# tulip-control/polytope

Measured on AMD Instinct MI355X. Metric: LP solves/sec (batched Chebyshev + redundancy), higher is better.
Workload: dtype f64

## Files before the change

### polytope_amd/csrc/plp_bbox_lane.hip

```cpp
#include "plp_reduce_lane.hpp"

namespace plp {

template <int D>
static int launch_bbox_lane_d(long long B, int m_max, const double* A, const double* b, const int* mrows, double* lb, double* ub,
                              int* status, hipStream_t st, double* xfin) {
    if (B > 2147483647ll) return 1;
    const int force = 0;
    const bool wide = m_max > LN_ROWS;
    int gs = wide ? (B <= PLP_REDUCE_LANE32_GS16_MAXB ? 16 : 8) : (B <= PLP_REDUCE_LANE_GS16_MAXB ? 16 : (B <= PLP_REDUCE_LANE_GS8_MAXB ? 8 : 4));
    const long long ng = 64 / gs;
    long long blocks = (B + ng - 1) / ng;
    if (blocks < 1) blocks = 1;
#define PLP_BBL(GSV, RV)                                                                                                     \
    hipLaunchKernelGGL((bbox_lane_kernel<D, GSV, RV>), dim3((unsigned)blocks), dim3(RBLOCK), reduce_lane_smem_bytes(D, GSV, RV), st, B, \
                       m_max, A, b, mrows, force, lb, ub, status, xfin)
    if (wide) { if (gs == 16) PLP_BBL(16, 32); else PLP_BBL(8, 32); }
    else if (gs == 16) PLP_BBL(16, 16);
    else if (gs == 8) PLP_BBL(8, 16);
    else PLP_BBL(4, 16);
#undef PLP_BBL
    return 0;
}

int launch_bbox_lane(long long B, int m_max, int d, const double* A, const double* b, const int* mrows, double* lb, double* ub,
                     int* status, hipStream_t st, double* xfin) {
    if (m_max < 1 || m_max > 2 * LN_ROWS) return 1;
    switch (d) {
        case 1: return launch_bbox_lane_d<1>(B, m_max, A, b, mrows, lb, ub, status, st, xfin);
        case 2: return launch_bbox_lane_d<2>(B, m_max, A, b, mrows, lb, ub, status, st, xfin);
        case 3: return launch_bbox_lane_d<3>(B, m_max, A, b, mrows, lb, ub, status, st, xfin);
        default: return 1;
    }
}

}
```

### polytope_amd/csrc/plp_kernels.hpp

```cpp
#pragma once
#include "plp_common.hpp"

namespace plp {

static inline int group_size_for(int m_max) {
    if (m_max < 0 || m_max > MAX_M) return -1;
    if (m_max <= 8) return 8;
    if (m_max <= 16) return 16;
    if (m_max <= 32) return 32;
    return 64;
}

int launch_lp(long long B, int m_max, int n, const double* c, const double* G, const double* h, const int* mrows,
              double* x, double* fun, int* status, int* iters, hipStream_t st);
int launch_lp_phase(long long B, int m_max, int n, const double* c, const double* G, const double* h, const int* mrows,
                    double* x, double* fun, int* status, int* iters, hipStream_t st, int phase, int* more);

int launch_cheby(long long B, int m_max, int d, const double* A, const double* b, const int* mrows, double* r,
                 double* xc, int* status, hipStream_t st);

int launch_lp_lds(long long B, int m_max, int n, const double* c, const double* G, const double* h, const int* mrows,
                  double* x, double* fun, int* status, int* iters, hipStream_t st);
int launch_cheby_lds(long long B, int m_max, int d, const double* A, const double* b, const int* mrows, double* r,
                     double* xc, int* status, hipStream_t st);
size_t lds_lp_bytes(int m_max, int nc);

int launch_cheby_gather_r(int d, long long n0, long long n1, long long n2, const int* off, const int* rows, const int* sel,
                          const double* A, const double* b, double* out, hipStream_t st);
int launch_rdiff_server(int d, int nwg, const unsigned long long* mail, const int* rec, void* out, unsigned long long* alive,
                        unsigned long long* dstate, const double* A, const double* b, unsigned long long last_word,
                        unsigned idle_polls, hipStream_t st);
void launch_rdiff_publish(long long n, const double* src, double* host_out, unsigned long long* host_flag,
                          unsigned long long seq, hipStream_t st);
int launch_cheby_gather_w(int d, long long nlp, const int* off, const int* rows, const int* sel, const double* A,
                          const double* b, double* out, hipStream_t st);
int launch_cheby_gather_lds(int d, int m_cap, long long nlp, const int* off, const int* rows, const int* sel,
                            const double* A, const double* b, double* out, hipStream_t st);

int launch_fm(int emit, long long B, int m_max, int d, const double* A, const double* b, const int* mrows,
              const unsigned long long* keep, int kw, const int* flags, int col, int first, double abs_tol, int* count,
              int mo_max, double* Aout, double* bout, int* mout, hipStream_t st);
size_t fm_lds_bytes(int m_max, int d);
int launch_volume_hits(long long B, int m_max, int d, const double* A, const double* b, const int* mrows, const double* lb,
                       const double* ub, const unsigned long long* state, const unsigned long long* inc, long long N,
                       unsigned* hits, int* flags, hipStream_t st);
int launch_support(long long B, int m_max, int d, const double* A, const double* b, const int* mrows, int K, const double* C,
                   int c_shared, const double* xc, double* val, double* x, int* status, hipStream_t st);
int launch_reduce_lds(long long B, int m_max, int d, const double* A, const double* b, const int* mrows, double abs_tol,
                      unsigned long long* keep, int* flags, double* r, double* xc, int* nlp, hipStream_t st);

int launch_cheby_w(long long B, int m_max, int d, const double* A, const double* b, const int* mrows, double* r,
                   double* xc, int* status, hipStream_t st);

int launch_lp_w(long long B, int m_max, int n, const double* c, const double* G, const double* h, const int* mrows,
                double* x, double* fun, int* status, int* iters, hipStream_t st);

int launch_lp_r(long long B, int m_max, int n, const double* c, const double* G, const double* h, const int* mrows,
                double* x, double* fun, int* status, int* iters, hipStream_t st);

int launch_cheby_r(long long B, int m_max, int d, const double* A, const double* b, const int* mrows, double* r,
                   double* xc, int* status, hipStream_t st);

struct BoxHandover {
    signed char* basis8;
    double* centre;
    double* xfin;
    int mode;
};
int launch_bbox(long long B, int m_max, int d, const double* A, const double* b, const int* mrows, double* lb,
                double* ub, int* status, hipStream_t st, BoxHandover* ho = nullptr);
int launch_bbox_lazy(long long B, int m_max, int d, const double* A, const double* b, const int* mrows, double* lb,
                     double* ub, int* status, hipStream_t st, BoxHandover* ho = nullptr);

int launch_adjacent(int n, int m_max, int d, const double* A, const double* b, const int* mrows, double inflate,
                    double thresh, unsigned char* adj, long long p_lo, long long p_hi, unsigned char* compact,
                    hipStream_t st, int cross_n1 = 0);

int launch_adjacent_w(int n, int m_max, int d, const double* A, const double* b, const int* mrows, double inflate,
                      double thresh, unsigned char* adj, long long p_lo, long long p_hi, unsigned char* compact,
                      hipStream_t st, int cross_n1 = 0);

struct ReduceArgs {
    long long B;
    int m_max;
    const double* A;
    const double* b;
    const int* mrows;
    double abs_tol;
    unsigned long long* keep;
    int* flags;
    double* r;
    double* xc;
    int* nlp;
    unsigned long long* ctr;
    unsigned long long* retry_word;
    unsigned long long epoch;
};
int launch_reduce(int d, const ReduceArgs& a, int phase, hipStream_t st);

int launch_contains(int P, int m_max, int d, const double* A, const double* b, const int* mrows, long long N,
                    const double* X, double abs_tol, int mode, unsigned char* out, void* scratch, hipStream_t st);
size_t contains_scratch_bytes(int P, int m_max);

int launch_assign(long long N, int d, const double* X, int F, const double* normals, const double* offsets,
                  double abs_tol, int* facet_of_point, double* dist, long long* argmax, double* maxd,
                  void* scratch, size_t scratch_bytes, hipStream_t st);
size_t assign_scratch_bytes(long long N, int F);

int launch_hull_reassign(long long N, int d, const double* X, int* owner, double* dist, const unsigned char* dead,
                         int new_id0, int n_new, const double* normals, const double* offsets, double abs_tol,
                         long long* argmax, double* maxd, long long* count, hipStream_t st);
void launch_hull_mark(int n, const int* ids, unsigned char* dead, hipStream_t st);
void launch_hull_drop(long long n, const long long* idx, int* owner, hipStream_t st);

int launch_selftest(int gs, double* out_d, unsigned* out_u, hipStream_t st);

size_t verify_scratch_bytes(long long nlp, int m_max);
bool verify_enabled();
int launch_verify_lp(long long B, int m_max, int n, const double* c, const double* G, const double* h, const int* mrows,
                     double* x, double* fun, int* status, void* scratch, int parity, hipStream_t st);
int launch_verify_cheby(long long B, int m_max, int d, const double* A, const double* b, const int* mrows, double* r,
                        double* xc, int* status, void* scratch, int parity, hipStream_t st);
int launch_verify_box(long long B, int m_max, int d, const double* A, const double* b, const int* mrows, double* lb, double* ub,
                      int* status, const signed char* basis8, const double* centre, const double* xfin, void* scratch,
                      int parity, hipStream_t st);

}
```

### polytope_amd/csrc/plp_lane_lp.hpp

```cpp
#pragma once
#include <math.h>

#if defined(__HIPCC__)
#include "plp_common.hpp"
#define PLP_LANE_FN __device__ __forceinline__
#else
#define PLP_LANE_FN static inline
namespace plp {
enum : int { ST_OPT = 0, ST_ITER = 1, ST_INFEAS = 2, ST_UNBND = 3, ST_NUM = 4 };
constexpr int ST_RETRY = 5;
constexpr double TOL_D = 1e-9, TOL_PIV = 1e-7, DEGEN_EPS = 1e-12;
constexpr int BLAND_AFTER = 6;
}
#endif

namespace plp {
namespace lane {

constexpr int LANE_MAX_ITERS = 48;
constexpr double LANE_TOL_D = 1e-11, LANE_TOL_PIV = 1e-11;
constexpr double LANE_M_NOISE = 64 * 2.220446049250313e-16;

struct Lp3 {
    double x0, x1, x2;
    int w0, w1, w2;
    int nact;
    int status;
    int iters;
    int ndeg;
};

PLP_LANE_FN void cross3(double a0, double a1, double a2, double b0, double b1, double b2, double& e0, double& e1,
                        double& e2) {
    e0 = fma(a1, b2, -(a2 * b1));
    e1 = fma(a2, b0, -(a0 * b2));
    e2 = fma(a0, b1, -(a1 * b0));
}

PLP_LANE_FN double dot3(double a0, double a1, double a2, double b0, double b1, double b2) {
    return fma(a2, b2, fma(a1, b1, a0 * b0));
}

template <class AnyF>
PLP_LANE_FN void proj1(const double c0, const double c1, const double c2, const double cn1, const double n0, const double n1,
                       const double n2, const double nn, double& d0, double& d1, double& d2, double& scale, AnyF ANY) {
    const double cn = dot3(c0, c1, c2, n0, n1, n2);
    d0 = fma(cn, n0, -(nn * c0));
    d1 = fma(cn, n1, -(nn * c1));
    d2 = fma(cn, n2, -(nn * c2));
    scale = nn;
    const double pn1 = fabs(d0) + fabs(d1) + fabs(d2);
    const bool small = (pn1 > 0.0) & (pn1 < 1e-4 * (nn * cn1));
    if (ANY(small)) {
        const double np_ = dot3(n0, n1, n2, d0, d1, d2);
        const double q0 = fma(nn, d0, -(np_ * n0)), q1 = fma(nn, d1, -(np_ * n1)), q2 = fma(nn, d2, -(np_ * n2));
        d0 = small ? q0 : d0;
        d1 = small ? q1 : d1;
        d2 = small ? q2 : d2;
        scale = small ? nn * nn : nn;
    }
}

constexpr double LANE_PAIR_SIN2 = 1e-10;

template <class RowF, class RatioF, class Ratio0F, class AnyF>
PLP_LANE_FN void walk3(Lp3& S, const double c0, const double c1, const double c2, const bool go, RowF ROWS, RatioF RATIO,
                       Ratio0F RATIO0, AnyF ANY, const bool warm = false) {
    if (!warm) {
        S.x0 = S.x1 = S.x2 = 0.0;
        S.w0 = S.w1 = S.w2 = -1;
        S.nact = 0;
        S.iters = 0;
        S.ndeg = 0;
    }
    S.status = go ? -1 : ST_OPT;
    const double cn1 = fabs(c0) + fabs(c1) + fabs(c2);
    if (go && !(cn1 > 0.0)) S.status = ST_OPT;
    if (!warm && ANY(S.status < 0)) {
        const bool step = S.status < 0;
        const double d0 = -c0, d1 = -c1, d2 = -c2;
        const double tolp = LANE_TOL_PIV * cn1;
        double bs = 1.0, bd = 0.0;
        int bi = -1;
        RATIO0(d0, d1, d2, tolp, bs, bd, bi);
        if (step) {
            S.iters = 1;
            if (bi < 0) {
                S.status = ST_UNBND;
            } else {
                const double t = bs / bd;
                S.x0 = fma(t, d0, 0.0);
                S.x1 = fma(t, d1, 0.0);
                S.x2 = fma(t, d2, 0.0);
                S.w0 = bi;
                S.nact = 1;
                S.ndeg = (t * cn1 <= DEGEN_EPS) ? 1 : 0;
            }
        }
    }
    while (ANY(S.status < 0)) {
        const bool run = S.status < 0;
        double d0 = -c0, d1 = -c1, d2 = -c2;
        double n00 = 0, n01 = 0, n02 = 0, n10 = 0, n11 = 0, n12 = 0, n20 = 0, n21 = 0, n22 = 0;
        if (ANY(run && S.nact >= 1)) {
            if (S.nact >= 1) ROWS(S.w0, n00, n01, n02);
            if (S.nact >= 2) ROWS(S.w1, n10, n11, n12);
            if (S.nact >= 3) ROWS(S.w2, n20, n21, n22);
        }
        bool stalled = false;
        double dscale = cn1;
        if (S.nact == 1) {
            const double nn = dot3(n00, n01, n02, n00, n01, n02);
            double sc;
            proj1(c0, c1, c2, cn1, n00, n01, n02, nn, d0, d1, d2, sc, ANY);
            dscale = sc * cn1;
        } else if (S.nact == 2) {
            double e0, e1, e2;
            cross3(n00, n01, n02, n10, n11, n12, e0, e1, e2);
            const double ce = dot3(c0, c1, c2, e0, e1, e2);
            d0 = -(ce * e0);
            d1 = -(ce * e1);
            d2 = -(ce * e2);
            dscale = dot3(e0, e1, e2, e0, e1, e2) * cn1;
            const double nn0 = dot3(n00, n01, n02, n00, n01, n02), nn1 = dot3(n10, n11, n12, n10, n11, n12);
            if (run && !(dot3(e0, e1, e2, e0, e1, e2) > LANE_PAIR_SIN2 * nn0 * nn1)) S.status = ST_RETRY;
        } else if (S.nact == 3) {
            d0 = d1 = d2 = 0.0;
        }
        {
            const double dn1 = fabs(d0) + fabs(d1) + fabs(d2);
            stalled = !(dn1 > LANE_TOL_D * dscale);
        }
        if (ANY(S.status < 0 && stalled)) {
            if (S.status < 0 && stalled) {
                if (S.nact == 0) {
                    S.status = ST_OPT;
                } else if (S.nact == 1) {
                    const double cn = dot3(c0, c1, c2, n00, n01, n02);
                    if (cn <= 0.0) S.status = ST_OPT;
                    else { S.nact = 0; d0 = -c0; d1 = -c1; d2 = -c2; }
                } else if (S.nact == 2) {
                    const double g00 = dot3(n00, n01, n02, n00, n01, n02), g11 = dot3(n10, n11, n12, n10, n11, n12);
                    const double g01 = dot3(n00, n01, n02, n10, n11, n12);
                    const double r0 = -dot3(c0, c1, c2, n00, n01, n02), r1 = -dot3(c0, c1, c2, n10, n11, n12);
                    const double l0 = fma(r0, g11, -(r1 * g01)), l1 = fma(r1, g00, -(r0 * g01));
                    const double w0 = 0.5 * (1.0 + g00), w1 = 0.5 * (1.0 + g11);
                    const double tol0 = LANE_TOL_D * g11 * w0 * cn1, tol1 = LANE_TOL_D * g00 * w1 * cn1;
                    if (l0 >= -tol0 && l1 >= -tol1) S.status = ST_OPT;
                    else {
                        const bool drop0 = l0 * w0 < l1 * w1;
                        if (drop0) { S.w0 = S.w1; n00 = n10; n01 = n11; n02 = n12; }
                        S.nact = 1;
                        double sc;
                        proj1(c0, c1, c2, cn1, n00, n01, n02, dot3(n00, n01, n02, n00, n01, n02), d0, d1, d2, sc, [](bool q) { return q; });
                    }
                } else {
                    double u00, u01, u02, u10, u11, u12, u20, u21, u22;
                    cross3(n10, n11, n12, n20, n21, n22, u00, u01, u02);
                    cross3(n20, n21, n22, n00, n01, n02, u10, u11, u12);
                    cross3(n00, n01, n02, n10, n11, n12, u20, u21, u22);
                    const double det = dot3(n00, n01, n02, u00, u01, u02);
                    const double g00 = dot3(n00, n01, n02, n00, n01, n02), g11 = dot3(n10, n11, n12, n10, n11, n12);
                    const double g22 = dot3(n20, n21, n22, n20, n21, n22);
                    if (!(det * det > 1e-18 * (g00 * g11 * g22))) {
                        S.status = ST_RETRY;
                    } else {
                        const double sg = det > 0.0 ? 1.0 : -1.0;
                        const double l0 = -sg * dot3(c0, c1, c2, u00, u01, u02);
                        const double l1 = -sg * dot3(c0, c1, c2, u10, u11, u12);
                        const double l2 = -sg * dot3(c0, c1, c2, u20, u21, u22);
                        const double a0 = l0 * (0.5 * (1.0 + g00)), a1 = l1 * (0.5 * (1.0 + g11)), a2 = l2 * (0.5 * (1.0 + g22));
                        const double tol = LANE_TOL_D * fabs(det) * cn1;
                        if (a0 >= -tol && a1 >= -tol && a2 >= -tol) S.status = ST_OPT;
                        else {
                            int j = 0;
                            double am = a0;
                            if (a1 < am) { am = a1; j = 1; }
                            if (a2 < am) { am = a2; j = 2; }
                            double gg;
                            if (j == 0) { d0 = -sg * u00; d1 = -sg * u01; d2 = -sg * u02; S.w0 = S.w1; S.w1 = S.w2; gg = g11 * g22; }
                            else if (j == 1) { d0 = -sg * u10; d1 = -sg * u11; d2 = -sg * u12; S.w1 = S.w2; gg = g22 * g00; }
                            else { d0 = -sg * u20; d1 = -sg * u21; d2 = -sg * u22; gg = g00 * g11; }
                            S.nact = 2;
                            if (!(dot3(d0, d1, d2, d0, d1, d2) > LANE_PAIR_SIN2 * gg)) S.status = ST_RETRY;
                        }
                    }
                }
            }
        }
        const bool step = S.status < 0;
        const double dn1 = fabs(d0) + fabs(d1) + fabs(d2);
        const double tolp = LANE_TOL_PIV * dn1;
        double bs = 1.0, bd = 0.0;
        int bi = -1;
        if (ANY(step)) RATIO(d0, d1, d2, S.x0, S.x1, S.x2, tolp, bs, bd, bi);
        if (step) {
            ++S.iters;
            if (bi < 0) {
                S.status = ST_UNBND;
            } else {
                const double t = bs / bd;
                S.x0 = fma(t, d0, S.x0);
                S.x1 = fma(t, d1, S.x1);
                S.x2 = fma(t, d2, S.x2);
                if (S.nact == 0) S.w0 = bi;
                else if (S.nact == 1) S.w1 = bi;
                else S.w2 = bi;
                S.nact += 1;
                S.ndeg = (t * dn1 <= DEGEN_EPS) ? S.ndeg + 1 : 0;
                if (S.ndeg >= BLAND_AFTER || S.iters >= LANE_MAX_ITERS) S.status = ST_RETRY;
            }
        }
    }
}

template <class RowF, class RatioF, class AnyF>
PLP_LANE_FN void walk3(Lp3& S, const double c0, const double c1, const double c2, const bool go, RowF ROWS, RatioF RATIO,
                       AnyF ANY, const bool warm = false) {
    walk3(S, c0, c1, c2, go, ROWS, RATIO,
          [&](double d0, double d1, double d2, double tolp, double& bs, double& bd, int& bi) {
              RATIO(d0, d1, d2, 0.0, 0.0, 0.0, tolp, bs, bd, bi);
          },
          ANY, warm);
}

struct Lp4 {
    double x0, x1, x2, x3;
    int w0, w1, w2, w3;
    int nact, status, iters, ndeg;
};

PLP_LANE_FN double dot4(double a0, double a1, double a2, double a3, double b0, double b1, double b2, double b3) {
    return fma(a3, b3, fma(a2, b2, fma(a1, b1, a0 * b0)));
}

PLP_LANE_FN void gcross4(double p0, double p1, double p2, double p3, double q0, double q1, double q2, double q3, double r0,
                         double r1, double r2, double r3, double& e0, double& e1, double& e2, double& e3) {
    const double m01 = fma(q0, r1, -(q1 * r0)), m02 = fma(q0, r2, -(q2 * r0)), m03 = fma(q0, r3, -(q3 * r0));
    const double m12 = fma(q1, r2, -(q2 * r1)), m13 = fma(q1, r3, -(q3 * r1)), m23 = fma(q2, r3, -(q3 * r2));
    e0 = fma(p1, m23, fma(-p2, m13, p3 * m12));
    e1 = -fma(p0, m23, fma(-p2, m03, p3 * m02));
    e2 = fma(p0, m13, fma(-p1, m03, p3 * m01));
    e3 = -fma(p0, m12, fma(-p1, m02, p2 * m01));
}

template <class RowF, class RatioF, class AnyF>
PLP_LANE_FN void walk4(Lp4& S, const double c0, const double c1, const double c2, const double c3, const bool go, RowF ROWS,
                       RatioF RATIO, AnyF ANY) {
    S.x0 = S.x1 = S.x2 = S.x3 = 0.0;
    S.w0 = S.w1 = S.w2 = S.w3 = -1;
    S.nact = 0;
    S.iters = 0;
    S.ndeg = 0;
    S.status = go ? -1 : ST_OPT;
    const double cn1 = fabs(c0) + fabs(c1) + fabs(c2) + fabs(c3);
    if (go && !(cn1 > 0.0)) S.status = ST_OPT;
    while (ANY(S.status < 0)) {
        const bool run = S.status < 0;
        bool dropped = false;
        double d0 = -c0, d1 = -c1, d2 = -c2, d3 = -c3;
        double n00 = 0, n01 = 0, n02 = 0, n03 = 0, n10 = 0, n11 = 0, n12 = 0, n13 = 0;
        double n20 = 0, n21 = 0, n22 = 0, n23 = 0, n30 = 0, n31 = 0, n32 = 0, n33 = 0;
        if (ANY(run && S.nact >= 1)) {
            if (S.nact >= 1) ROWS(S.w0, n00, n01, n02, n03);
            if (S.nact >= 2) ROWS(S.w1, n10, n11, n12, n13);
            if (S.nact >= 3) ROWS(S.w2, n20, n21, n22, n23);
            if (S.nact >= 4) ROWS(S.w3, n30, n31, n32, n33);
        }
        const double g00 = dot4(n00, n01, n02, n03, n00, n01, n02, n03), g11 = dot4(n10, n11, n12, n13, n10, n11, n12, n13);
        const double g22 = dot4(n20, n21, n22, n23, n20, n21, n22, n23);
        const double g01 = dot4(n00, n01, n02, n03, n10, n11, n12, n13), g02 = dot4(n00, n01, n02, n03, n20, n21, n22, n23);
        const double g12 = dot4(n10, n11, n12, n13, n20, n21, n22, n23);
        const double r0 = dot4(c0, c1, c2, c3, n00, n01, n02, n03), r1 = dot4(c0, c1, c2, c3, n10, n11, n12, n13);
        const double r2 = dot4(c0, c1, c2, c3, n20, n21, n22, n23);
        double det = 1.0, m0 = 0.0, m1 = 0.0, m2 = 0.0;
        if (S.nact == 1) {
            det = g00;
            m0 = r0;
        } else if (S.nact == 2) {
            det = fma(g00, g11, -(g01 * g01));
            m0 = fma(r0, g11, -(r1 * g01));
            m1 = fma(r1, g00, -(r0 * g01));
            if (run && !(det > LANE_PAIR_SIN2 * g00 * g11)) S.status = ST_RETRY;
        } else if (S.nact == 3) {
            const double A00 = fma(g11, g22, -(g12 * g12)), A01 = fma(g02, g12, -(g01 * g22)), A02 = fma(g01, g12, -(g02 * g11));
            const double A11 = fma(g00, g22, -(g02 * g02)), A12 = fma(g01, g02, -(g00 * g12)), A22 = fma(g00, g11, -(g01 * g01));
            det = fma(g00, A00, fma(g01, A01, g02 * A02));
            m0 = fma(A00, r0, fma(A01, r1, A02 * r2));
            m1 = fma(A01, r0, fma(A11, r1, A12 * r2));
            m2 = fma(A02, r0, fma(A12, r1, A22 * r2));
            if (run && !(det > 1e-16 * g00 * g11 * g22)) S.status = ST_RETRY;
        }
        bool twice = false;
        if (S.nact == 3) {
            double e0, e1, e2, e3;
            gcross4(n00, n01, n02, n03, n10, n11, n12, n13, n20, n21, n22, n23, e0, e1, e2, e3);
            const double ce = dot4(c0, c1, c2, c3, e0, e1, e2, e3);
            d0 = -(ce * e0);
            d1 = -(ce * e1);
            d2 = -(ce * e2);
            d3 = -(ce * e3);
        } else if (S.nact >= 1 && S.nact <= 2) {
            d0 = fma(m1, n10, fma(m0, n00, -(det * c0)));
            d1 = fma(m1, n11, fma(m0, n01, -(det * c1)));
            d2 = fma(m1, n12, fma(m0, n02, -(det * c2)));
            d3 = fma(m1, n13, fma(m0, n03, -(det * c3)));
            if (S.nact == 1) {
                const double nd = dot4(n00, n01, n02, n03, d0, d1, d2, d3);
                d0 = fma(g00, d0, -(nd * n00));
                d1 = fma(g00, d1, -(nd * n01));
                d2 = fma(g00, d2, -(nd * n02));
                d3 = fma(g00, d3, -(nd * n03));
            } else {
                const double dn = fabs(d0) + fabs(d1) + fabs(d2) + fabs(d3);
                twice = (dn > 0.0) & (dn < 1e-4 * (det * cn1));
                if (ANY(run && twice)) {
                    const double s0 = dot4(d0, d1, d2, d3, n00, n01, n02, n03), s1 = dot4(d0, d1, d2, d3, n10, n11, n12, n13);
                    const double k0 = fma(s0, g11, -(s1 * g01)), k1 = fma(s1, g00, -(s0 * g01));
                    const double q0 = fma(det, d0, -fma(k1, n10, k0 * n00)), q1 = fma(det, d1, -fma(k1, n11, k0 * n01));
                    const double q2 = fma(det, d2, -fma(k1, n12, k0 * n02)), q3 = fma(det, d3, -fma(k1, n13, k0 * n03));
                    d0 = twice ? q0 : d0;
                    d1 = twice ? q1 : d1;
                    d2 = twice ? q2 : d2;
                    d3 = twice ? q3 : d3;
                }
            }
        } else if (S.nact == 4) {
            d0 = d1 = d2 = d3 = 0.0;
        }
        const double dscale = (S.nact >= 1 && S.nact <= 3) ? ((S.nact == 1 || twice) ? det * det : det) * cn1 : cn1;
        const bool stalled = !(fabs(d0) + fabs(d1) + fabs(d2) + fabs(d3) > LANE_TOL_D * dscale);
        if (ANY(S.status < 0 && stalled)) {
            if (S.status < 0 && stalled) {
                const double w0 = 0.5 * (1.0 + g00), w1 = 0.5 * (1.0 + g11), w2 = 0.5 * (1.0 + g22);
                if (S.nact == 0) {
                    S.status = ST_OPT;
                } else if (S.nact <= 3) {
                    const double tol = LANE_TOL_D * det * cn1;
                    double f0 = 0.0, f1 = 0.0, f2 = 0.0;
                    if (S.nact == 2) {
                        f0 = fabs(r0 * g11) + fabs(r1 * g01);
                        f1 = fabs(r1 * g00) + fabs(r0 * g01);
                    } else if (S.nact == 3) {
                        const double B00 = fabs(g11 * g22) + g12 * g12, B01 = fabs(g02 * g12) + fabs(g01 * g22), B02 = fabs(g01 * g12) + fabs(g02 * g11);
                        const double B11 = fabs(g00 * g22) + g02 * g02, B12 = fabs(g01 * g02) + fabs(g00 * g12), B22 = fabs(g00 * g11) + g01 * g01;
                        f0 = B00 * fabs(r0) + B01 * fabs(r1) + B02 * fabs(r2);
                        f1 = B01 * fabs(r0) + B11 * fabs(r1) + B12 * fabs(r2);
                        f2 = B02 * fabs(r0) + B12 * fabs(r1) + B22 * fabs(r2);
                    }
                    const double a0 = -m0 * w0, a1 = S.nact >= 2 ? -m1 * w1 : 0.0, a2 = S.nact >= 3 ? -m2 * w2 : 0.0;
                    const double t0 = fmax(tol, LANE_M_NOISE * f0 * w0), t1 = fmax(tol, LANE_M_NOISE * f1 * w1), t2 = fmax(tol, LANE_M_NOISE * f2 * w2);
                    if (a0 >= -t0 && a1 >= -t1 && a2 >= -t2) {
                        S.status = ST_OPT;
                    } else {
                        int j = 0;
                        double am = a0 + t0;
                        if (a1 + t1 < am) { am = a1 + t1; j = 1; }
                        if (a2 + t2 < am) { am = a2 + t2; j = 2; }
                        if (j == 0) S.w0 = S.w1;
                        if (j <= 1) S.w1 = S.w2;
                        S.nact -= 1;
                        dropped = true;
                    }
                } else {
                    const double g33 = dot4(n30, n31, n32, n33, n30, n31, n32, n33);
                    const double w3 = 0.5 * (1.0 + g33);
                    double am = 0.0, bd0 = 0.0, bd1 = 0.0, bd2 = 0.0, bd3 = 0.0, dj_abs = 0.0;
                    int jbest = -1;
                    bool all_ok = true, singular = false;
#define PLP_W4_VERTEX(J, P, Q, R, NJ0, NJ1, NJ2, NJ3, WJ)                                                          \
                    {                                                                                                   \
                        double u0, u1, u2, u3;                                                                          \
                        gcross4(P##0, P##1, P##2, P##3, Q##0, Q##1, Q##2, Q##3, R##0, R##1, R##2, R##3, u0, u1, u2, u3); \
                        const double dj = dot4(NJ0, NJ1, NJ2, NJ3, u0, u1, u2, u3);                                     \
                        const double sg = dj > 0.0 ? 1.0 : -1.0;                                                        \
                        const double lj = -sg * dot4(c0, c1, c2, c3, u0, u1, u2, u3);                                   \
                        const double aj = lj * (WJ);                                                                    \
                        dj_abs = fabs(dj);                                                                              \
                        singular = singular | !(dj * dj > 1e-18 * (g00 * g11 * g22 * g33));                            \
                        all_ok = all_ok & (aj >= -(LANE_TOL_D * dj_abs * cn1));                                              \
                        const bool better = (jbest < 0) | (aj < am);                                                    \
                        am = better ? aj : am;                                                                          \
                        jbest = better ? (J) : jbest;                                                                   \
                        bd0 = better ? -sg * u0 : bd0;                                                                  \
                        bd1 = better ? -sg * u1 : bd1;                                                                  \
                        bd2 = better ? -sg * u2 : bd2;                                                                  \
                        bd3 = better ? -sg * u3 : bd3;                                                                  \
                    }
                    PLP_W4_VERTEX(0, n1, n2, n3, n00, n01, n02, n03, w0)
                    PLP_W4_VERTEX(1, n0, n2, n3, n10, n11, n12, n13, w1)
                    PLP_W4_VERTEX(2, n0, n1, n3, n20, n21, n22, n23, w2)
                    PLP_W4_VERTEX(3, n0, n1, n2, n30, n31, n32, n33, w3)
#undef PLP_W4_VERTEX
                    if (singular) S.status = ST_RETRY;
                    else if (all_ok) S.status = ST_OPT;
                    else {
                        d0 = bd0; d1 = bd1; d2 = bd2; d3 = bd3;
                        if (jbest == 0) S.w0 = S.w1;
                        if (jbest <= 1) S.w1 = S.w2;
                        if (jbest <= 2) S.w2 = S.w3;
                        S.nact = 3;
                    }
                }
            }
        }
        if (dropped) {
            ++S.iters;
            if (S.iters >= LANE_MAX_ITERS) S.status = ST_RETRY;
        }
        const bool step = (S.status < 0) & !dropped;
        const double dn1 = fabs(d0) + fabs(d1) + fabs(d2) + fabs(d3);
        const double tolp = LANE_TOL_PIV * dn1;
        double bs = 1.0, bd = 0.0;
        int bi = -1;
        if (ANY(step)) RATIO(d0, d1, d2, d3, S.x0, S.x1, S.x2, S.x3, tolp, bs, bd, bi);
        if (step) {
            ++S.iters;
            if (bi < 0) {
                S.status = ST_UNBND;
            } else {
                const double t = bs / bd;
                S.x0 = fma(t, d0, S.x0);
                S.x1 = fma(t, d1, S.x1);
                S.x2 = fma(t, d2, S.x2);
                S.x3 = fma(t, d3, S.x3);
                if (S.nact == 0) S.w0 = bi;
                else if (S.nact == 1) S.w1 = bi;
                else if (S.nact == 2) S.w2 = bi;
                else S.w3 = bi;
                S.nact += 1;
                S.ndeg = (t * dn1 <= DEGEN_EPS) ? S.ndeg + 1 : 0;
                if (S.ndeg >= BLAND_AFTER || S.iters >= LANE_MAX_ITERS) S.status = ST_RETRY;
            }
        }
    }
}

PLP_LANE_FN void ratio_row4(const double a0, const double a1, const double a2, const double a3, const double beta, const int i,
                            const double d0, const double d1, const double d2, const double d3, const double x0,
                            const double x1, const double x2, const double x3, const double tolp, double& bs, double& bd,
                            int& bi) {
    const double ad = dot4(a0, a1, a2, a3, d0, d1, d2, d3);
    const double ax = dot4(a0, a1, a2, a3, x0, x1, x2, x3);
    const double sl = fmax(beta - ax, 0.0);
    const bool better = (ad > tolp) & (sl * bd < bs * ad);
    bs = better ? sl : bs;
    bd = better ? ad : bd;
    bi = better ? i : bi;
}

PLP_LANE_FN void ratio_row(const double a0, const double a1, const double a2, const double beta, const int i, const double d0,
                           const double d1, const double d2, const double x0, const double x1, const double x2,
                           const double tolp, double& bs, double& bd, int& bi) {
    const double ad = dot3(a0, a1, a2, d0, d1, d2);
    const double ax = dot3(a0, a1, a2, x0, x1, x2);
    const double sl = fmax(beta - ax, 0.0);
    const bool better = (ad > tolp) & (sl * bd < bs * ad);
    bs = better ? sl : bs;
    bd = better ? ad : bd;
    bi = better ? i : bi;
}

PLP_LANE_FN void ratio_row0(const double a0, const double a1, const double a2, const double beta, const int i, const double d0,
                            const double d1, const double d2, const double tolp, double& bs, double& bd, int& bi) {
    const double ad = dot3(a0, a1, a2, d0, d1, d2);
    const double sl = fmax(beta, 0.0);
    const bool better = (ad > tolp) & (sl * bd < bs * ad);
    bs = better ? sl : bs;
    bd = better ? ad : bd;
    bi = better ? i : bi;
}

template <int M, class RowF, class BetaF, class AnyF, class PassF>
PLP_LANE_FN void solve3(Lp3& S, const double c0, const double c1, const double c2, const bool go, RowF ROWS, BetaF BETA,
                        AnyF ANY, PassF PASS, const bool warm = false) {
    walk3(S, c0, c1, c2, go, ROWS,
          [&](double d0, double d1, double d2, double x0, double x1, double x2, double tolp, double& bs, double& bd, int& bi) {
              PASS();
#pragma unroll
              for (int i = 0; i < M; ++i) {
                  double a0, a1, a2;
                  ROWS(i, a0, a1, a2);
                  ratio_row(a0, a1, a2, BETA(i), i, d0, d1, d2, x0, x1, x2, tolp, bs, bd, bi);
              }
          },
          ANY, warm);
}

template <int M, class RowF, class BetaF, class AnyF>
PLP_LANE_FN void solve3(Lp3& S, const double c0, const double c1, const double c2, const bool go, RowF ROWS, BetaF BETA,
                        AnyF ANY, const bool warm = false) {
    solve3<M>(S, c0, c1, c2, go, ROWS, BETA, ANY, [] {}, warm);
}

}
}
```

### polytope_amd/csrc/plp_reduce.hip

```cpp
#include "plp_kernels.hpp"
#include "plp_reduce_plan.hpp"

namespace plp {

template <int D>
int launch_reduce_d(const ReduceLaunch& L, const ReduceArgs& a, int force, int retry_only, hipStream_t st);

static int launch_plan(int d, const ReduceLaunch& L, const ReduceArgs& a, int force, int retry_only, hipStream_t st) {
    switch (d) {
#define PLP_CASE_D(K) \
    case K: return launch_reduce_d<K>(L, a, force, retry_only, st);
        PLP_CASE_D(1) PLP_CASE_D(2) PLP_CASE_D(3) PLP_CASE_D(4) PLP_CASE_D(5) PLP_CASE_D(6) PLP_CASE_D(7) PLP_CASE_D(8)
        PLP_CASE_D(9) PLP_CASE_D(10) PLP_CASE_D(11) PLP_CASE_D(12) PLP_CASE_D(13) PLP_CASE_D(14) PLP_CASE_D(15) PLP_CASE_D(16)
#undef PLP_CASE_D
        default: return 2;
    }
}

int launch_reduce(int d, const ReduceArgs& a, int phase, hipStream_t st) {
    const ReducePlan p = plan_reduce(a.B, a.m_max, d, reduce_env());
    if (p.first.engine == RE_NONE) return 2;
    if (phase != 2) {
        const int rc = launch_plan(d, p.first, a, p.force_retry, 0, st);
        if (rc || !p.second || phase == 1) return rc;
    }
    return launch_plan(d, p.retry, a, p.force_retry, 1, st);
}

}
```

### polytope_amd/csrc/plp_reduce_d1_4.hip

```cpp
#include "plp_reduce_launch.hpp"

namespace plp {

PLP_REDUCE_INSTANTIATE(1)
PLP_REDUCE_INSTANTIATE(2)
PLP_REDUCE_INSTANTIATE(3)
PLP_REDUCE_INSTANTIATE(4)

}

#ifdef PLP_STAGE_STATS
extern "C" __attribute__((visibility("default"))) int plp_debug_stage_stats(unsigned long long* out16, int reset) {
    (void)hipDeviceSynchronize();
    if (out16 && hipMemcpyFromSymbol(out16, HIP_SYMBOL(plp::plp_stage_stats), 128) != hipSuccess) return 1;
    if (reset) {
        unsigned long long z[16] = {0};
        if (hipMemcpyToSymbol(HIP_SYMBOL(plp::plp_stage_stats), z, 128) != hipSuccess) return 1;
    }
    return 0;
}
#endif
```

### polytope_amd/csrc/plp_reduce_lane.hpp

```cpp
#pragma once
#include <type_traits>

#include "plp_lane_lp.hpp"
#include "plp_reduce_general.hpp"
#include "plp_reduce_r_impl.hpp"

namespace plp {

#ifndef PLP_LANE_CH
#define PLP_LANE_CH 4
#endif

constexpr int LN_ROWS = 16;

template <int D, int GS, int ROWS>
__device__ __noinline__ void reduce_lane_redo(unsigned char* smem_raw, const long long tile, const int ntile, const uint64_t rb64,
                                              int m_max, const double* __restrict__ Ag, const double* __restrict__ bg,
                                              const int* __restrict__ mrows, double abs_tol,
                                              unsigned long long* __restrict__ keep_out, int* __restrict__ flags_out,
                                              double* __restrict__ r_out, double* __restrict__ xc_out,
                                              int* __restrict__ nlp_out) {
    constexpr int PER = 64 / ROWS;
    for (int sub = 0; sub < (64 / GS) / PER; ++sub) {
        unsigned some = 0u;
#pragma unroll
        for (int q = 0; q < PER; ++q) some |= (unsigned)((rb64 >> (GS * (PER * sub + q))) & 1ull) << q;
        if (some == 0u) continue;
        const int q = (threadIdx.x & 63) / ROWS;
        const bool mine = ((some >> q) & 1u) != 0u;
        const int left = ntile - PER * sub;
        reduce_general_tile<D, RBLOCK>(smem_raw, tile + PER * sub, left < PER ? left : PER, mine, m_max, ROWS, Ag, bg, mrows, abs_tol,
                                       keep_out, flags_out, r_out, xc_out, nlp_out);
    }
}

template <int D, int GS, int ROWS = LN_ROWS, bool BBOX = false>
__device__ __forceinline__ void reduce_lane_tile(
    const long long tile, long long B, int m_max, const double* __restrict__ Ag, const double* __restrict__ bg,
    const int* __restrict__ mrows, double abs_tol, int force_retry, unsigned long long* __restrict__ keep_out,
    int* __restrict__ flags_out, double* __restrict__ r_out, double* __restrict__ xc_out, int* __restrict__ nlp_out,
    unsigned long long* __restrict__ ctr) {
    static_assert(D >= 1 && D <= 4, "the lane engine walks in R^3 (lower dimensions are embedded) or R^4");
    static_assert(RBLOCK == 64, "one wavefront per workgroup");
    static_assert(GS == 4 || GS == 8 || GS == 16, "lanes per polytope");
    static_assert((ROWS == 16 || ROWS == 32) && ROWS / GS >= 1 && ROWS / GS <= 4, "row slots per polytope, at most four per lane");
    constexpr int rows = ROWS, R = rows / GS, NG = 64 / GS;
    constexpr unsigned RMASK = (1u << R) - 1u;
    constexpr int LS = NG;
    extern __shared__ __attribute__((aligned(16))) unsigned char smem_raw[];
    const Grp g(GS);
    const int lane = g.lane;
    const int gib = lane / GS;
    const int row0 = g.gl * R;
    double* sA = reinterpret_cast<double*>(smem_raw);
    double* sb = sA + (size_t)rows * D * NG;
    double* san = sb + (size_t)rows * NG;
    double* myA = sA + gib;
    constexpr int OFF_B = rows * D * NG, OFF_N = OFF_B + rows * NG;
    double* const myb = myA + OFF_B;
    double* const myan = myA + OFF_N;
#define LA(i, kk) myA[((i) * D + (kk)) * LS]
#define LB(i) myA[OFF_B + (i) * LS]
#define LN(i) myA[OFF_N + (i) * LS]
    double* const rA = myA + row0 * D * LS;
    double* const rS = myA + row0 * LS;
#define OA(k, kk) rA[((k) * D + (kk)) * LS]
#define OB(k) rS[OFF_B + (k) * LS]
#define ON(k) rS[OFF_N + (k) * LS]
    const double qnan = __longlong_as_double(0x7ff8000000000000ll);
    const double pinf = __longlong_as_double(0x7ff0000000000000ll);
    const int ntile = (B - tile) < NG ? (int)(B - tile) : NG;
    __syncthreads();
    {
        const int p = lane % NG, q = lane / NG;
        const int rowsz = m_max * D;
        const bool pv = p < ntile;
        const double* src = Ag + (tile + (pv ? p : 0)) * rowsz;
        double va[rows * D / GS], vb[rows / GS];
        const double* srcb = bg + (tile + (pv ? p : 0)) * m_max;
        if (m_max == rows) {
#pragma unroll
            for (int it = 0; it < rows * D / GS; ++it) va[it] = src[q + GS * it];
#pragma unroll
            for (int it = 0; it < rows / GS; ++it) vb[it] = srcb[q + GS * it];
        } else {
#pragma unroll
            for (int it = 0; it < rows * D / GS; ++it) {
                const int rem = q + GS * it;
                va[it] = src[rem < rowsz ? rem : 0];
            }
#pragma unroll
            for (int it = 0; it < rows / GS; ++it) {
                const int row = q + GS * it;
                vb[it] = srcb[row < m_max ? row : 0];
            }
        }
#pragma unroll
        for (int it = 0; it < rows * D / GS; ++it) {
            const int rem = q + GS * it;
            sA[rem * NG + p] = (pv & (rem < rowsz)) ? va[it] : 0.0;
        }
#pragma unroll
        for (int it = 0; it < rows / GS; ++it) {
            const int row = q + GS * it;
            sb[row * NG + p] = (pv & (row < m_max)) ? vb[it] : 0.0;
        }
    }
    __syncthreads();
    const bool valid = gib < ntile;
    const int m = valid ? (mrows ? (mrows + tile)[gib] : m_max) : 0;
    double xc[D];
    double rr = 0.0;
    bool ball, fulldim, f1open = false;
    uint64_t live = 0ull;
    unsigned has = 0u;
    bool retry = force_retry != 0;
    {
        SimplexR<D + 1, R, false, true> S;
        double qi[R];
        S.reset(D + 1, m, row0);
        unsigned actb = 0u;
        bool inf0 = false, finite = true;
#pragma unroll
        for (int k = 0; k < R; ++k) {
            const bool h = valid & (row0 + k < m) & (m <= rows);
            has |= h ? (1u << k) : 0u;
            double nrm2 = 0.0;
#pragma unroll
            for (int kk = 0; kk < D; ++kk) {
                const double v = h ? OA(k, kk) : 0.0;
                S.T[k][kk] = v;
                nrm2 = nrm2 + v * v;
                finite = finite & isfinite(v);
            }
            const double bk = h ? OB(k) : 0.0;
            finite = finite & isfinite(bk);
            const double nrm = sqrt(nrm2);
            ON(k) = 1.0 / nrm;
            const bool zero = !(nrm > 0.0);
            const bool on = h & !zero;
            S.T[k][D] = on ? nrm : 0.0;
            S.beta[k] = on ? bk : 0.0;
            qi[k] = bk / nrm;
            actb |= on ? (1u << k) : 0u;
            inf0 = inf0 | (h & zero & (bk < -TOL_FEAS));
        }
        S.ract = actb;
        const bool infeasible0 = grp_ballot(inf0, g) != 0;
        const bool bad = (grp_ballot(!finite, g) != 0) | (m > rows);
        S.cost[D] = -1.0;
        S.mode = M_P2;
        if (!valid | bad) { S.mode = M_DONE; S.status = ST_NUM; }
        else if (infeasible0) { S.mode = M_DONE; S.status = ST_INFEAS; }
#ifndef PLP_LANE_DBG_NOF1
        S.template run_fast<GS, true>(g, qi, actb);
#endif
        retry = retry | (valid & (S.status == ST_RETRY));
        const bool ok = S.status == ST_OPT;
        f1open = valid & !ok & (S.status != ST_INFEAS);
#pragma unroll
        for (int j = 0; j <= D; ++j) {
            bool found;
            const double mine = S.x_of(j, found);
            const uint64_t ob = grp_ballot(found, g);
            const double v = bcast(mine, g.gbase + (ob ? __ffsll((long long)ob) - 1 : 0));
            const double xj = ob ? v : 0.0;
            if (j < D) xc[j < D ? j : 0] = xj; else rr = xj;
        }
        ball = ok & (rr >= 0.0);
        fulldim = ball & (rr > abs_tol);
        if constexpr (BBOX) fulldim = ball & (rr >= 1e-6);
    }
    if (!BBOX && (valid & (g.gl == 0))) {
        (r_out + tile)[gib] = ball ? rr : 0.0;
#pragma unroll
        for (int k = 0; k < D; ++k) (xc_out + tile * D)[gib * D + k] = ball ? xc[k] : qnan;
    }
    __syncthreads();
#ifdef PLP_LANE_DBG_F1ONLY
    if (valid & (g.gl == 0)) { (keep_out + tile)[gib] = 0; (flags_out + tile)[gib] = 0; (nlp_out + tile)[gib] = 1; }
    return;
#endif
    if constexpr (BBOX) {
#pragma unroll
        for (int k = 0; k < R; ++k) live |= spread_rows<R, GS>(grp_ballot(((has >> k) & 1u) != 0u, g)) << k;
    } else {
        unsigned remmask = 0u;
        const double scr_thr = sqrt(2.0 * abs_tol) * 1.0001 + 1e-12;
        double ni[R][D], bin_[R];
#pragma unroll
        for (int k = 0; k < R; ++k) {
            const double an_i = ON(k);
#pragma unroll
            for (int kk = 0; kk < D; ++kk) ni[k][kk] = OA(k, kk) * an_i;
            bin_[k] = OB(k) * an_i;
        }
#pragma unroll 2
        for (int t = 1; t <= rows / 2; ++t) {
#pragma unroll
            for (int k = 0; k < R; ++k) {
                const int i = row0 + k;
                const int j = (i + t) & (rows - 1);
                const double an_j = LN(j);
                if (!__any(fabs(ni[k][0] - LA(j, 0) * an_j) < scr_thr)) continue;
                double dot = 0.0;
#pragma unroll
                for (int kk = 0; kk < D; ++kk) dot = dot + ni[k][kk] * (LA(j, kk) * an_j);
                const double bjn = LB(j) * an_j;
                const bool par = valid & (m <= rows) & (i < m) & (j < m) & (dot > 1.0 - abs_tol);
                const bool i_lo = i < j;
                const double blo = i_lo ? bin_[k] : bjn, bhi = i_lo ? bjn : bin_[k];
                const int lo = i_lo ? i : j, hi = i_lo ? j : i;
                const int gone = (blo < bhi) ? hi : lo;
                remmask |= par ? (1u << gone) : 0u;
            }
        }
#pragma unroll
        for (int o = 1; o < GS; o <<= 1) remmask |= (unsigned)__shfl_xor((int)remmask, o, 64);
        const unsigned removed = (remmask >> row0) & RMASK;
#pragma unroll
        for (int k = 0; k < R; ++k)
            live |= spread_rows<R, GS>(grp_ballot((((has & ~removed) >> k) & 1u) != 0u, g)) << k;
    }
    bool neg = false;
#pragma unroll
    for (int k = 0; k < R; ++k) {
        double sk = 0.0;
#pragma unroll
        for (int kk = 0; kk < D; ++kk) sk = fma(((has >> k) & 1u) ? OA(k, kk) : 0.0, ball ? xc[kk] : 0.0, sk);
        const double raw = (((has >> k) & 1u) ? OB(k) : 0.0) - sk;
        neg = neg | (raw < 0.0);
        ON(k) = fmax(raw, 0.0);
    }
    if (__any(neg & ball)) {
        bool off = false;
        const double xs = centre_scale<D>(xc);
#pragma unroll
        for (int k = 0; k < R; ++k) {
            const bool hk = ((has >> k) & 1u) != 0u;
            double sk = 0.0, nrm2 = 0.0;
#pragma unroll
            for (int kk = 0; kk < D; ++kk) {
                const double v = hk ? OA(k, kk) : 0.0;
                sk = fma(v, ball ? xc[kk] : 0.0, sk);
                nrm2 = nrm2 + v * v;
            }
            const double bk = hk ? OB(k) : 0.0;
            off = off | (hk & centre_off(bk - sk, 1.0 / sqrt(nrm2), bk, xs));
        }
        if (ball & (grp_ballot(off, g) != 0)) {
            ball = false; fulldim = false; f1open = true;
            if (!BBOX && (valid & (g.gl == 0))) {
                (r_out + tile)[gib] = 0.0;
#pragma unroll
                for (int k = 0; k < D; ++k) (xc_out + tile * D)[gib * D + k] = qnan;
            }
        }
    }
    auto zero_dead = [&](unsigned alive) {
#pragma unroll
        for (int k = 0; k < R; ++k) {
            if (!((alive >> k) & 1u)) {
#pragma unroll
                for (int kk = 0; kk < D; ++kk) OA(k, kk) = 0.0;
                OB(k) = 0.0;
                ON(k) = 0.0;
            }
        }
    };
    zero_dead(((unsigned)(live >> row0) & RMASK));
    int flags = fulldim ? 0 : (RF_EMPTY | (f1open ? RF_F1OPEN : 0));
    int nlp = 1;
    uint64_t keep = 0ull;
    int stage = 0;
    if (fulldim) {
        const int neq = __popcll(live);
        if (neq <= D + 1) { flags = RF_EARLY; keep = live; }
        else stage = (neq > 3 * D) ? 1 : 2;
        if constexpr (BBOX) stage = 1;
    }
    __syncthreads();
    auto any_lane = [](bool p) { return __any(p) != 0; };
    using LpState = std::conditional_t<D == 4, lane::Lp4, lane::Lp3>;
    auto lane_solve = [&](LpState& S, const double (&cv)[4], const bool go_, const double* pA, const double* pbeta, auto relax_tag,
                          int krv, const int nparts, const int part) {
        constexpr bool RELAX = decltype(relax_tag)::value;
        const int cnt = rows / nparts;
        const int i0 = part * cnt;
        auto row_of = [&](const double* base, double& a0, double& a1, double& a2, double& a3) {
            a0 = base[0];
            a1 = D > 1 ? base[(D > 1 ? 1 : 0) * LS] : 0.0;
            a2 = D > 2 ? base[(D > 2 ? 2 : 0) * LS] : 0.0;
            a3 = D > 3 ? base[(D > 3 ? 3 : 0) * LS] : 0.0;
        };
        auto ratio = [&](auto x0_tag, const double (&dv)[4], const double (&xv)[4], double tolp, double& bs, double& bd, int& bi) {
            constexpr bool X0 = decltype(x0_tag)::value;
            if constexpr (RELAX) asm volatile("" : "+v"(krv));
            const double* ra = pA + i0 * D * LS;
            const double* rb_ = pbeta + i0 * LS;
            int ic = i0;
            for (int ch = 0; ch < cnt; ch += PLP_LANE_CH) {
#pragma unroll
                for (int r = 0; r < PLP_LANE_CH; ++r) {
                    double a0, a1, a2, a3;
                    row_of(ra + (r * D) * LS, a0, a1, a2, a3);
                    double beta = rb_[r * LS];
                    if constexpr (RELAX) beta = beta + ((ic + r == krv) ? 0.1 : 0.0);
                    if constexpr (D == 4)
                        lane::ratio_row4(a0, a1, a2, a3, beta, ic + r, dv[0], dv[1], dv[2], dv[3], xv[0], xv[1], xv[2], xv[3], tolp,
                                         bs, bd, bi);
                    else if constexpr (X0)
                        lane::ratio_row0(a0, a1, a2, beta, ic + r, dv[0], dv[1], dv[2], tolp, bs, bd, bi);
                    else
                        lane::ratio_row(a0, a1, a2, beta, ic + r, dv[0], dv[1], dv[2], xv[0], xv[1], xv[2], tolp, bs, bd, bi);
                }
                ra += PLP_LANE_CH * D * LS;
                rb_ += PLP_LANE_CH * LS;
                ic += PLP_LANE_CH;
            }
            auto meet = [&](auto ctrl) {
                constexpr int CTRL = decltype(ctrl)::value;
                const double ps = dpp_d<CTRL>(bs), pd = dpp_d<CTRL>(bd);
                const int pi = dpp_i<CTRL>(bi);
                const double l = ps * bd, r_ = bs * pd;
                const bool theirs = (pd > 0.0) & (!(bd > 0.0) | (l < r_) | ((l == r_) & (pi < bi)));
                bs = theirs ? ps : bs;
                bd = theirs ? pd : bd;
                bi = theirs ? pi : bi;
            };
            if (nparts > 1) meet(std::integral_constant<int, PLP_DPP_XOR1>{});
            if (nparts > 2) meet(std::integral_constant<int, PLP_DPP_XOR2>{});
        };
        if constexpr (D == 4) {
            lane::walk4(
                S, cv[0], cv[1], cv[2], cv[3], go_,
                [&](int i, double& a0, double& a1, double& a2, double& a3) { row_of(pA + (i * D) * LS, a0, a1, a2, a3); },
                [&](double d0, double d1, double d2, double d3, double x0, double x1, double x2, double x3, double tolp, double& bs,
                    double& bd, int& bi) {
                    const double dv[4] = {d0, d1, d2, d3}, xv[4] = {x0, x1, x2, x3};
                    ratio(std::false_type{}, dv, xv, tolp, bs, bd, bi);
                },
                any_lane);
        } else {
            lane::walk3(
                S, cv[0], cv[1], cv[2], go_,
                [&](int i, double& a0, double& a1, double& a2) {
                    double a3;
                    row_of(pA + (i * D) * LS, a0, a1, a2, a3);
                },
                [&](double d0, double d1, double d2, double x0, double x1, double x2, double tolp, double& bs, double& bd, int& bi) {
                    const double dv[4] = {d0, d1, d2, 0.0}, xv[4] = {x0, x1, x2, 0.0};
                    ratio(std::false_type{}, dv, xv, tolp, bs, bd, bi);
                },
                [&](double d0, double d1, double d2, double tolp, double& bs, double& bd, int& bi) {
                    const double dv[4] = {d0, d1, d2, 0.0}, xv[4] = {0.0, 0.0, 0.0, 0.0};
                    ratio(std::true_type{}, dv, xv, tolp, bs, bd, bi);
                },
                any_lane);
        }
    };
    auto x_of_lp = [](const LpState& S, int k) {
        double v = k == 0 ? S.x0 : (k == 1 ? S.x1 : S.x2);
        if constexpr (D == 4) v = k == 3 ? S.x3 : v;
        return v;
    };
#ifdef PLP_LANE_DBG_NOF3
    if (false) {
#else
    if (__any(stage == 1)) {
#endif
        const bool go = stage == 1;
        const unsigned lloc = ((unsigned)(live >> row0) & RMASK);
        bool lpfail = false;
        constexpr int NLP = 2 * D;
        constexpr int NROUND = GS == 16 ? 1 : (NLP + GS - 1) / GS;
        auto f3_pair = [](int rd) { return GS == 16 || 2 * (NLP - rd * GS < GS ? NLP - rd * GS : GS) <= GS; };
        auto f3_round_of = [](int it) { return GS == 16 ? 0 : it / GS; };
        auto f3_lane_of = [&](int it) { const int rd = f3_round_of(it); return f3_pair(rd) ? 2 * (it - rd * GS) : it - rd * GS; };
        double val[NROUND];
#pragma unroll
        for (int q = 0; q < NROUND; ++q) val[q] = 0.0;
#pragma unroll 1
        for (int rd = 0; rd < NROUND; ++rd) {
            const bool pair = f3_pair(rd);
            const int nparts = pair ? 2 : 1;
            const int it = rd * GS + (pair ? (g.gl >> 1) : g.gl);
            const int part = pair ? (g.gl & 1) : 0;
            const bool mine = go & (it < 2 * D);
            const int kx = it >> 1;
            const bool up = it & 1;
            const double cs = up ? -1.0 : 1.0;
            LpState S;
            const double cv[4] = {kx == 0 ? cs : 0.0, kx == 1 ? cs : 0.0, kx == 2 ? cs : 0.0, kx == 3 ? cs : 0.0};
            lane_solve(S, cv, mine, myA, myan, std::false_type{}, -1, nparts, part);
            double xck = 0.0;
#pragma unroll
            for (int kk = 0; kk < D; ++kk) xck = (kk == kx) ? xc[kk] : xck;
            const double xk = x_of_lp(S, kx);
            double v;
            if (S.status == ST_OPT) v = xck + xk;
            else if (S.status == ST_UNBND) v = up ? pinf : -pinf;
            else { v = qnan; lpfail = lpfail | (mine & (S.status != ST_RETRY)); }
            retry = retry | (mine & (S.status == ST_RETRY));
            if constexpr (BBOX) {
                double* xfin = reinterpret_cast<double*>(keep_out);
                if (xfin && (valid & mine & (part == 0))) {
#pragma unroll
                    for (int kk = 0; kk < D; ++kk) xfin[((size_t)(tile + gib) * 2 * D + it) * D + kk] = xc[kk] + x_of_lp(S, kk);
                }
            }
#pragma unroll
            for (int q = 0; q < NROUND; ++q) val[q] = (q == rd) ? v : val[q];
        }
        lpfail = grp_ballot(lpfail, g) != 0;
        retry = retry | (grp_ballot(retry, g) != 0);
        if constexpr (BBOX) {
#pragma unroll
            for (int it2 = 0; it2 < NLP; ++it2) {
                const double v = bcast(val[f3_round_of(it2)], g.gbase + f3_lane_of(it2));
                if (valid & (g.gl == 0)) ((it2 & 1) ? xc_out + tile * D : r_out + tile * D)[gib * D + (it2 >> 1)] = go ? v : qnan;
            }
            if (valid & (g.gl == 0)) (flags_out + tile)[gib] = (go & !retry & !lpfail) ? 0 : 1;
            return;
        }
        double s1[R], s2[R];
#pragma unroll
        for (int k = 0; k < R; ++k) { s1[k] = 0.0; s2[k] = 0.0; }
#pragma unroll
        for (int kx = 0; kx < D; ++kx) {
            const int itl = 2 * kx, ith = 2 * kx + 1;
            const double lo = bcast(val[f3_round_of(itl)], g.gbase + f3_lane_of(itl));
            const double hi = bcast(val[f3_round_of(ith)], g.gbase + f3_lane_of(ith));
#pragma unroll
            for (int k = 0; k < R; ++k) {
                const double aik = OA(k, kx);
                const double pa = (aik > 0.0 ? 1.0 : 0.0) * aik;
                s1[k] = s1[k] + pa * (hi - lo);
                s2[k] = s2[k] + aik * lo;
            }
        }
        uint64_t outb = 0ull;
#pragma unroll
        for (int k = 0; k < R; ++k) {
            const bool out = go & (((lloc >> k) & 1u) != 0u) & ((s1[k] - (OB(k) - s2[k])) < -1e-4);
            outb |= spread_rows<R, GS>(grp_ballot(out, g)) << k;
        }
        __syncthreads();
        if (go) {
            live = live & ~outb;
            zero_dead(((unsigned)(live >> row0) & RMASK));
            nlp += 2 * D;
            if (lpfail) flags |= RF_LPFAIL;
            if (__popcll(live) <= D + 1) { flags |= RF_EARLY; keep = live; stage = 0; }
            else stage = 2;
        }
        __syncthreads();
    }
    if constexpr (BBOX) {
        if (valid & (g.gl == 0)) {
            (flags_out + tile)[gib] = 1;
#pragma unroll
            for (int k = 0; k < D; ++k) { (r_out + tile * D)[gib * D + k] = qnan; (xc_out + tile * D)[gib * D + k] = qnan; }
        }
        return;
    }
#ifdef PLP_LANE_DBG_NOF2
    if (false) {
#else
    if (__any(stage == 2)) {
#endif
        const unsigned lloc = ((unsigned)(live >> row0) & RMASK);
        uint64_t todo = (stage == 2) ? live : 0ull;
        if (stage == 2) nlp += __popcll(live);
#ifndef PLP_LANE_DBG_NOPRE
        {
            const unsigned okb = f2_presolve<D, R, LS, true>(myA, myb, myan, row0, m_max, (stage == 2) ? lloc : 0u, abs_tol);
            uint64_t cert = 0ull;
#pragma unroll
            for (int k = 0; k < R; ++k) cert |= spread_rows<R, GS>(grp_ballot(((okb >> k) & 1u) != 0u, g)) << k;
            keep |= cert;
            todo &= ~cert;
            ctr_add(ctr, -__popcll(cert), g.gl == 0);
        }
#endif
        __syncthreads();
        const unsigned todo32 = (unsigned)todo;
        const int n_g = __popc(todo32);
        int total = 0, nmax = 0;
        for (int p = 0; p < NG; ++p) {
            const int np = __builtin_amdgcn_readlane(n_g, p * GS);
            total += np;
            nmax = np > nmax ? np : nmax;
        }
        int off_g = 0;
        for (int p = 0, run = 0; p < NG; ++p) {
            off_g = (gib == p) ? run : off_g;
            run += __builtin_amdgcn_readlane(n_g, p * GS);
        }
        unsigned retry_polys = 0u;
        int rb = 0;
        while (rb < total) {
            const int nrem = total - rb;
            const int nparts = nrem <= 16 ? 4 : (nrem <= 32 ? 2 : 1);
            const int sh = nparts == 4 ? 2 : (nparts == 2 ? 1 : 0);
            const int per = 64 >> sh;
            const int t = rb + (lane >> sh);
            const int part = lane & (nparts - 1);
            int tp = 0, toff = 0, run = 0;
            unsigned ttd = 0u;
            for (int p = 0; p < NG; ++p) {
                const int np = __builtin_amdgcn_readlane(n_g, p * GS);
                const unsigned tdp = (unsigned)__builtin_amdgcn_readlane((int)todo32, p * GS);
                const bool at = t >= run;
                tp = at ? p : tp;
                ttd = at ? tdp : ttd;
                toff = at ? run : toff;
                run += np;
            }
            const bool mine = t < total;
            {
                const int rank = t - toff;
                for (int i = 0; i < nmax; ++i) ttd = (i < rank) ? (ttd & (ttd - 1u)) : ttd;
            }
            const int kr = mine ? (__ffs((int)ttd) - 1) : 0;
            const double* pA = sA + tp;
            const double* pan = pA + OFF_N;
            double c[4] = {0.0, 0.0, 0.0, 0.0};
#pragma unroll
            for (int kk = 0; kk < D; ++kk) c[kk] = -pA[(kr * D + kk) * LS];
            LpState S;
            lane_solve(S, c, mine, pA, pan, std::true_type{}, kr, nparts, part);
            double akx = -lane::dot3(c[0], c[1], c[2], S.x0, S.x1, S.x2);
            if constexpr (D == 4) akx = -lane::dot4(c[0], c[1], c[2], c[3], S.x0, S.x1, S.x2, S.x3);
            const double obj = akx - pan[kr * LS];
            const bool keepk = mine & (((S.status == ST_OPT) & (obj > abs_tol)) | (S.status == ST_UNBND));
            const uint64_t all = __ballot(keepk);
            const uint64_t rt = __ballot(mine & (S.status == ST_RETRY));
            if (rt != 0ull) {
                for (int p = 0; p < NG; ++p)
                    if (__any(mine & (S.status == ST_RETRY) & (tp == p))) retry_polys |= 1u << p;
            }
#pragma unroll
            for (int k = 0; k < R; ++k) {
                const int rw = row0 + k;
                const int tt = off_g + __popc(todo32 & ((1u << rw) - 1u)) - rb;
                const bool own = (((todo32 >> rw) & 1u) != 0u) & (tt >= 0) & (tt < per);
                const bool kept = own & (((all >> ((tt << sh) & 63)) & 1ull) != 0ull);
                keep |= spread_rows<R, GS>(grp_ballot(kept, g)) << k;
            }
            rb += per;
        }
        retry = retry | (((retry_polys >> gib) & 1u) != 0u);
        if (stage == 2) flags |= RF_MINREP;
    }
    if (valid & (g.gl == 0) & !retry) {
        (keep_out + tile)[gib] = keep;
        (flags_out + tile)[gib] = flags;
        (nlp_out + tile)[gib] = nlp;
    }
    ctr_add(ctr, nlp, valid & (g.gl == 0));
    const uint64_t rb64 = __ballot(retry & valid & (g.gl == 0));
    if (rb64 != 0ull) {
        __threadfence_block();
        __syncthreads();
        reduce_lane_redo<D, GS, ROWS>(smem_raw, tile, ntile, rb64, m_max, Ag, bg, mrows, abs_tol, keep_out, flags_out, r_out, xc_out,
                            nlp_out);
    }
#undef LA
#undef OA
#undef OB
#undef ON
#undef LB
#undef LN
}

#ifndef PLP_REDUCE_LANE_WAVES
#define PLP_REDUCE_LANE_WAVES(D) ((D) <= 3 ? 4 : 3)
#endif

template <int D, int GS, int ROWS = LN_ROWS>
__global__ __launch_bounds__(RBLOCK, PLP_REDUCE_LANE_WAVES(D)) void reduce_lane_kernel(
    long long B, int m_max, const double* __restrict__ Ag, const double* __restrict__ bg, const int* __restrict__ mrows,
    double abs_tol, int force_retry, unsigned long long* __restrict__ keep_out, int* __restrict__ flags_out,
    double* __restrict__ r_out, double* __restrict__ xc_out, int* __restrict__ nlp_out, unsigned long long* __restrict__ ctr) {
    reduce_lane_tile<D, GS, ROWS>((long long)blockIdx.x * (64 / GS), B, m_max, Ag, bg, mrows, abs_tol, force_retry, keep_out,
                                  flags_out, r_out, xc_out, nlp_out, ctr);
}

template <int D, int ROWS, int GSA, int GSB>
__global__ __launch_bounds__(RBLOCK, PLP_REDUCE_LANE_WAVES(D)) void reduce_lane_mix_kernel(
    int nbig, long long B, int m_max, const double* __restrict__ Ag, const double* __restrict__ bg,
    const int* __restrict__ mrows, double abs_tol, int force_retry, unsigned long long* __restrict__ keep_out,
    int* __restrict__ flags_out, double* __restrict__ r_out, double* __restrict__ xc_out, int* __restrict__ nlp_out,
    unsigned long long* __restrict__ ctr) {
    constexpr int NA = 64 / GSA, NB_ = 64 / GSB;
    if ((int)blockIdx.x < nbig)
        reduce_lane_tile<D, GSA, ROWS>((long long)blockIdx.x * NA, B, m_max, Ag, bg, mrows, abs_tol, force_retry, keep_out,
                                       flags_out, r_out, xc_out, nlp_out, ctr);
    else
        reduce_lane_tile<D, GSB, ROWS>((long long)nbig * NA + (long long)((int)blockIdx.x - nbig) * NB_, B, m_max, Ag, bg, mrows,
                                       abs_tol, force_retry, keep_out, flags_out, r_out, xc_out, nlp_out, ctr);
}

template <int D, int GS, int ROWS>
__global__ __launch_bounds__(RBLOCK, PLP_REDUCE_LANE_WAVES(D)) void bbox_lane_kernel(
    long long B, int m_max, const double* __restrict__ Ag, const double* __restrict__ bg, const int* __restrict__ mrows,
    int force_retry, double* __restrict__ lb, double* __restrict__ ub, int* __restrict__ status, double* __restrict__ xfin) {
    reduce_lane_tile<D, GS, ROWS, true>((long long)blockIdx.x * (64 / GS), B, m_max, Ag, bg, mrows, 0.0, force_retry,
                                        reinterpret_cast<unsigned long long*>(xfin), status, lb, ub, nullptr, nullptr);
}

}
```

### polytope_amd/csrc/plp_reduce_launch.hpp

```cpp
#pragma once
#include "plp_reduce_general.hpp"
#include "plp_reduce_lane.hpp"
#include "plp_reduce_plan.hpp"
#include "plp_reduce_r_impl.hpp"

namespace plp {

static_assert(REDUCE_GENERAL_BLOCK == BLOCK, "workgroup of the general kernel");

#define PLP_REDUCE_GO(KERNEL)                                                                                                   \
    hipLaunchKernelGGL(KERNEL, dim3((unsigned)L.grid), dim3(L.block), L.lds, st, a.B, a.m_max, a.A, a.b, a.mrows, a.abs_tol, \
                       force, a.keep, a.flags, a.r, a.xc, a.nlp, a.ctr, a.retry_word, a.epoch)

template <int D, int GS, int R>
static inline void reduce_go_group(const ReduceLaunch& L, const ReduceArgs& a, int force, hipStream_t st) {
    if (L.lds > 48 * 1024)
        (void)hipFuncSetAttribute(reinterpret_cast<const void*>(reduce_r_kernel<D, GS, R>),
                                  hipFuncAttributeMaxDynamicSharedMemorySize, (int)L.lds);
    PLP_REDUCE_GO((reduce_r_kernel<D, GS, R>));
}

#define PLP_REDUCE_GO_LANE(KERNEL)                                                                                              \
    hipLaunchKernelGGL(KERNEL, dim3((unsigned)L.grid), dim3(L.block), L.lds, st, a.B, a.m_max, a.A, a.b, a.mrows, a.abs_tol, \
                       force, a.keep, a.flags, a.r, a.xc, a.nlp, a.ctr)

template <int D>
int launch_reduce_d(const ReduceLaunch& L, const ReduceArgs& a, int force, int retry_only, hipStream_t st) {
    static_assert(sizeof(wide::WideShared<D + 1>) == wide_shared_bytes(D), "plan's LDS of the one-LP-per-wavefront engines");
    static_assert(reduce_lazy_smem_bytes(D) == reduce_r_smem_bytes(64, D, 1) + lazy::lds_bytes<D>(), "lazy LDS");
    switch (L.engine) {
        case RE_GENERAL:
            hipLaunchKernelGGL(reduce_kernel<D>, dim3((unsigned)L.grid), dim3(L.block), L.lds, st, a.B, a.m_max, L.gs, a.A, a.b,
                               a.mrows, a.abs_tol, retry_only, a.keep, a.flags, a.r, a.xc, a.nlp,
                               retry_only ? a.retry_word : nullptr, a.epoch);
            return 0;
        case RE_LANE:
            if constexpr (D <= 4) {
                if (L.rows == 32) {
                    if (L.gs == 16) PLP_REDUCE_GO_LANE((reduce_lane_kernel<D, 16, 32>));
                    else PLP_REDUCE_GO_LANE((reduce_lane_kernel<D, 8, 32>));
                } else if (L.gs == 16) PLP_REDUCE_GO_LANE((reduce_lane_kernel<D, 16, 16>));
                else if (L.gs == 8) PLP_REDUCE_GO_LANE((reduce_lane_kernel<D, 8, 16>));
                else PLP_REDUCE_GO_LANE((reduce_lane_kernel<D, 4, 16>));
                return 0;
            }
            return 2;
        case RE_LANE_MIX:
            if constexpr (D <= 4) {
                if (L.rows == 32)
                    hipLaunchKernelGGL((reduce_lane_mix_kernel<D, 32, 8, 16>), dim3((unsigned)L.grid), dim3(L.block), L.lds, st,
                                       (int)L.nbig, a.B, a.m_max, a.A, a.b, a.mrows, a.abs_tol, force, a.keep, a.flags, a.r, a.xc,
                                       a.nlp, a.ctr);
                else
                    hipLaunchKernelGGL((reduce_lane_mix_kernel<D, 16, 4, 8>), dim3((unsigned)L.grid), dim3(L.block), L.lds, st,
                                       (int)L.nbig, a.B, a.m_max, a.A, a.b, a.mrows, a.abs_tol, force, a.keep, a.flags, a.r, a.xc,
                                       a.nlp, a.ctr);
                return 0;
            }
            return 2;
        case RE_GROUP:
            if constexpr (D <= 8) {
                if (L.rows == 4) {
                    if (L.gs == 4) reduce_go_group<D, 4, 4>(L, a, force, st);
                    else if (L.gs == 8) reduce_go_group<D, 8, 4>(L, a, force, st);
                    else reduce_go_group<D, 16, 4>(L, a, force, st);
                    return 0;
                }
                if constexpr (D >= 5) {
                    if (L.gs == 8) reduce_go_group<D, 8, 2>(L, a, force, st);
                    else if (L.gs == 16) reduce_go_group<D, 16, 2>(L, a, force, st);
                    else reduce_go_group<D, 32, 2>(L, a, force, st);
                    return 0;
                }
            } else {
                if (L.rows == 1) reduce_go_group<D, 64, 1>(L, a, force, st);
                else if (L.gs == 16) reduce_go_group<D, 16, 2>(L, a, force, st);
                else reduce_go_group<D, 32, 2>(L, a, force, st);
                return 0;
            }
            return 2;
        case RE_GROUP_MIX:
            if constexpr (D <= 4) {
                hipLaunchKernelGGL((reduce_r_mix_kernel<D>), dim3((unsigned)L.grid), dim3(L.block), L.lds, st, (int)L.nbig, a.B,
                                   a.m_max, a.A, a.b, a.mrows, a.abs_tol, force, a.keep, a.flags, a.r, a.xc, a.nlp, a.ctr,
                                   a.retry_word, a.epoch);
                return 0;
            }
            return 2;
        case RE_SPLIT:
            if constexpr (D <= 8) {
                if (L.gs == 4) PLP_REDUCE_GO((reduce_split_kernel<D, 4, 4>));
                else if (L.gs == 8) PLP_REDUCE_GO((reduce_split_kernel<D, 8, 4>));
                else PLP_REDUCE_GO((reduce_split_kernel<D, 16, 4>));
            } else {
                if (L.gs == 16) PLP_REDUCE_GO((reduce_split_kernel<D, 16, 2>));
                else PLP_REDUCE_GO((reduce_split_kernel<D, 32, 2>));
            }
            return 0;
        case RE_WDENSE:
        case RE_LAZY:
        case RE_WSPLIT:
            if constexpr (D >= 5) {
                if (L.engine == RE_WDENSE) PLP_REDUCE_GO((reduce_wdense_kernel<D>));
                else if (L.engine == RE_LAZY) PLP_REDUCE_GO((reduce_lazy_kernel<D>));
                else if (L.nw == 4) PLP_REDUCE_GO((reduce_wsplit_kernel<D, 4, (D <= PLP_REDUCE_WDENSE_MAXD)>));
                else PLP_REDUCE_GO((reduce_wsplit_kernel<D, 2, (D <= PLP_REDUCE_WDENSE_MAXD)>));
                return 0;
            }
            return 2;
        default:
            return 2;
    }
}

#undef PLP_REDUCE_GO
#undef PLP_REDUCE_GO_LANE

#define PLP_REDUCE_INSTANTIATE(D) \
    template int launch_reduce_d<D>(const ReduceLaunch&, const ReduceArgs&, int, int, hipStream_t);

}
```

### polytope_amd/csrc/plp_reduce_plan.hpp

```cpp
#pragma once
#include <stddef.h>
#include <stdlib.h>

namespace plp {

#ifndef PLP_REDUCE_R_BLOCK
#define PLP_REDUCE_R_BLOCK 64
#endif
constexpr int RBLOCK = PLP_REDUCE_R_BLOCK;
constexpr int REDUCE_GENERAL_BLOCK = 256;

#ifndef PLP_REDUCE_WG_MAXB
#define PLP_REDUCE_WG_MAXB 1500
#endif

#ifndef PLP_REDUCE_LANE_MINB
#define PLP_REDUCE_LANE_MINB 0
#endif
#ifndef PLP_REDUCE_LANE4_MINB
#define PLP_REDUCE_LANE4_MINB 40000
#endif
#ifndef PLP_REDUCE_LANE4_MINB_ROWS14
#define PLP_REDUCE_LANE4_MINB_ROWS14 3000
#endif

#ifndef PLP_REDUCE_LANE32_GS16_MAXB
#define PLP_REDUCE_LANE32_GS16_MAXB 16000
#endif
#ifndef PLP_REDUCE_LANE_GS8_MAXB
#define PLP_REDUCE_LANE_GS8_MAXB 40000
#endif
#ifndef PLP_REDUCE_LANE_GS16_MAXB
#define PLP_REDUCE_LANE_GS16_MAXB 14000
#endif
#define PLP_REDUCE_LANE_MIX_DIV 8
#define PLP_REDUCE_LANE_MIX_MAXTAIL 1024
#define PLP_REDUCE_LANE_MIX_MINBLOCKS 512

#ifndef PLP_REDUCE_SPLIT_MAXB
#define PLP_REDUCE_SPLIT_MAXB(D, GS) \
    ((((GS) == 4 && (D) >= 7) || (D) > 8 || ((D) >= 5 && (GS) == 16)) ? 1024 : ((D) >= 5 ? 2048 : 4096))
#endif

#define PLP_REDUCE_MIX_DIV 32
#define PLP_REDUCE_MIX_MAXTAIL 1024
#define PLP_REDUCE_MIX_MINBLOCKS 4096
#define PLP_REDUCE_HALF_MAXBLOCKS 2048

#ifndef PLP_REDUCE_WDENSE_MAXD
#define PLP_REDUCE_WDENSE_MAXD 13
#endif

#define PLP_REDUCE_WS2_MAXB_DENSE 16000
#define PLP_REDUCE_WS4_MAXB_DENSE8 12000
#define PLP_REDUCE_WS4_MAXB_DENSE 2000
#define PLP_REDUCE_WS2_MAXB_LAZY 3000
#define PLP_REDUCE_WS4_MAXB_LAZY 500

constexpr int reduce_general_gs(int m_max) { return m_max <= 8 ? 8 : (m_max <= 16 ? 16 : (m_max <= 32 ? 32 : 64)); }
constexpr size_t reduce_smem_bytes(int gs, int D) {
    return ((size_t)(REDUCE_GENERAL_BLOCK / gs) * gs * (D + 1) * 8 + 15) & ~(size_t)15;
}
constexpr int group_size_r(int m_max) { return m_max <= 16 ? 4 : (m_max <= 32 ? 8 : 16); }
constexpr size_t reduce_r_smem_bytes(int gs, int D, int R) {
    return ((size_t)(RBLOCK / gs) * gs * R * (D + 2) * 8 + 15) & ~(size_t)15;
}
constexpr size_t reduce_split_smem_bytes(int gs, int D, int R) {
    return (((size_t)gs * R * (D + 2) + 2 * D + 2) * 8 + 15) & ~(size_t)15;
}
constexpr size_t reduce_lane_smem_bytes(int D, int GS, int ROWS) { return (size_t)(64 / GS) * ROWS * (D + 2) * 8; }
constexpr size_t wide_shared_bytes(int D) { return ((size_t)20 * (D + 2) + 7) & ~(size_t)7; }
constexpr size_t reduce_lazy_smem_bytes(int D) {
    return reduce_r_smem_bytes(64, D, 1) + ((wide_shared_bytes(D) + 255) & ~(size_t)255);
}
constexpr size_t reduce_wsplit_smem_bytes(int D, int NW) {
    return (size_t)64 * (D + 2) * 8 + (size_t)(D + 2 + 2 * D) * 8 + 8 * 8 + 8 * 4 + 64 * 4 +
           NW * ((wide_shared_bytes(D) + 15) & ~(size_t)15) + (size_t)2 * NW * 8 + (size_t)NW * 64 * 4;
}

enum ReduceEngine : int {
    RE_NONE = 0,
    RE_GENERAL,
    RE_LANE,
    RE_LANE_MIX,
    RE_GROUP,
    RE_GROUP_MIX,
    RE_SPLIT,
    RE_WDENSE,
    RE_LAZY,
    RE_WSPLIT,
};

struct ReduceLaunch {
    int engine = RE_NONE;
    int gs = 0;
    int rows = 0;
    int nw = 0;
    int dense = 0;
    long long nbig = 0;
    long long grid = 0;
    int block = 0;
    size_t lds = 0;
};

struct ReducePlan {
    ReduceLaunch first;
    bool second = false;
    ReduceLaunch retry;
    int force_retry = 0;
};

struct ReduceEnv {
    const char* lane = nullptr;
    const char* lane_gs = nullptr;
    const char* lane_mix = nullptr;
    const char* retry_all = nullptr;
    const char* one_row = nullptr;
    const char* r1 = nullptr;
    const char* r2 = nullptr;
    const char* lazy = nullptr;
    const char* split = nullptr;
    const char* half = nullptr;
    const char* wsplit = nullptr;
    const char* wdense = nullptr;
};

inline ReduceEnv reduce_env() {
    ReduceEnv e;
    e.lane = getenv("PLP_REDUCE_LANE");
    e.lane_gs = getenv("PLP_REDUCE_LANE_GS");
    e.lane_mix = getenv("PLP_REDUCE_LANE_MIX");
    e.retry_all = getenv("PLP_REDUCE_RETRY_ALL");
    e.one_row = getenv("PLP_REDUCE_1ROW");
    e.r1 = getenv("PLP_REDUCE_R1");
    e.r2 = getenv("PLP_REDUCE_R2");
    e.lazy = getenv("PLP_REDUCE_LAZY");
    e.split = getenv("PLP_REDUCE_SPLIT");
    e.half = getenv("PLP_REDUCE_HALF");
    e.wsplit = getenv("PLP_REDUCE_WSPLIT");
    e.wdense = getenv("PLP_REDUCE_WDENSE");
    return e;
}

namespace plan_detail {

inline bool is(const char* s, char c) { return s && s[0] == c; }
inline long long cdiv(long long a, long long b) { return (a + b - 1) / b; }
inline long long at_least1(long long v) { return v < 1 ? 1 : v; }

inline ReduceLaunch launch(int engine, int gs, int rows, long long grid, int block, size_t lds) {
    ReduceLaunch L;
    L.engine = engine;
    L.gs = gs;
    L.rows = rows;
    L.grid = grid;
    L.block = block;
    L.lds = lds;
    return L;
}

inline bool plan_lane(long long B, int m_max, int d, const ReduceEnv& env, ReduceLaunch& L) {
    if (B > 2147483647ll) return false;
    const char* eg = env.lane_gs;
    const int rows = m_max > 16 ? 32 : 16;
    int gs;
    if (rows == 32) gs = eg ? (atoi(eg) == 16 ? 16 : 8) : (B <= PLP_REDUCE_LANE32_GS16_MAXB ? 16 : 8);
    else if (eg) gs = atoi(eg) == 16 ? 16 : (atoi(eg) == 8 ? 8 : 4);
    else gs = B <= PLP_REDUCE_LANE_GS16_MAXB ? 16 : (B <= PLP_REDUCE_LANE_GS8_MAXB ? 8 : 4);
    const long long ng = 64 / gs;
    const long long blocks = at_least1(cdiv(B, ng));
    L = launch(RE_LANE, gs, rows, blocks, RBLOCK, reduce_lane_smem_bytes(d, gs, rows));
    if (gs != (rows == 32 ? 8 : 4)) return true;
    long long tail = blocks / PLP_REDUCE_LANE_MIX_DIV < PLP_REDUCE_LANE_MIX_MAXTAIL ? blocks / PLP_REDUCE_LANE_MIX_DIV
                                                                                    : PLP_REDUCE_LANE_MIX_MAXTAIL;
    if (env.lane_mix) tail = blocks * atoi(env.lane_mix) / 64;
    if (eg || (rows == 32 && d == 4)) tail = 0;
    if (tail > 0 && blocks > PLP_REDUCE_LANE_MIX_MINBLOCKS) {
        L.engine = RE_LANE_MIX;
        L.nbig = blocks - tail;
        L.grid = L.nbig + cdiv(B - L.nbig * ng, ng / 2);
    }
    return true;
}

inline bool plan_lazy(long long B, int d, const ReduceEnv& env, ReduceLaunch& L, bool& complete) {
    if (B > 2147483647ll) return false;
    const bool dense = env.wdense ? env.wdense[0] == '1' : (d <= PLP_REDUCE_WDENSE_MAXD);
    complete = dense && !is(env.retry_all, '1');
    const long long maxb = dense ? PLP_REDUCE_WS2_MAXB_DENSE : PLP_REDUCE_WS2_MAXB_LAZY;
    const long long maxb4 = dense ? (d <= 8 ? PLP_REDUCE_WS4_MAXB_DENSE8 : PLP_REDUCE_WS4_MAXB_DENSE)
                                  : PLP_REDUCE_WS4_MAXB_LAZY;
    const char* ws = env.wsplit;
    int nw = 0;
    if (B >= 1 && !is(ws, '0')) {
        if (is(ws, '4') || (!ws && B <= maxb4)) nw = 4;
        else if (is(ws, '2') || (!ws && B <= maxb)) nw = 2;
    }
    if (nw && dense == (d <= PLP_REDUCE_WDENSE_MAXD)) {
        L = launch(RE_WSPLIT, 64, 1, B, 64 * nw, reduce_wsplit_smem_bytes(d, nw));
        L.nw = nw;
        L.dense = dense;
        return true;
    }
    L = launch(dense ? RE_WDENSE : RE_LAZY, 64, 1, at_least1(B), RBLOCK, reduce_lazy_smem_bytes(d));
    return true;
}

inline bool plan_group(long long B, int d, int GS, int R, const ReduceEnv& env, ReduceLaunch& L) {
    const long long NG = RBLOCK / GS;
    long long blocks = cdiv(B, NG);
    if (blocks > 2147483647ll) return false;
    blocks = at_least1(blocks);
    const size_t smem = reduce_r_smem_bytes(GS, d, R);
    if ((R == 4 && d <= 8) || (R == 2 && d > 8)) {
        if (is(env.split, '1') || (!is(env.split, '0') && B <= PLP_REDUCE_SPLIT_MAXB(d, GS))) {
            L = launch(RE_SPLIT, GS, R, at_least1(B), RBLOCK, reduce_split_smem_bytes(GS, d, R));
            return true;
        }
    }
    if (GS == 4 && R == 4 && d <= 4) {
        const size_t smem2 = reduce_r_smem_bytes(8, d, 2);
        const size_t smix = smem > smem2 ? smem : smem2;
        if (blocks <= 2 * PLP_REDUCE_HALF_MAXBLOCKS &&
            (is(env.half, '1') || (!is(env.half, '0') && blocks <= PLP_REDUCE_HALF_MAXBLOCKS))) {
            L = launch(RE_GROUP_MIX, GS, R, cdiv(B, NG / 2), RBLOCK, smix);
            return true;
        }
        if (blocks > PLP_REDUCE_MIX_MINBLOCKS) {
            const long long tail = blocks / PLP_REDUCE_MIX_DIV < PLP_REDUCE_MIX_MAXTAIL ? blocks / PLP_REDUCE_MIX_DIV
                                                                                      : PLP_REDUCE_MIX_MAXTAIL;
            L = launch(RE_GROUP_MIX, GS, R, 0, RBLOCK, smix);
            L.nbig = blocks - tail;
            L.grid = L.nbig + cdiv(B - L.nbig * NG, NG / 2);
            return true;
        }
    }
    L = launch(RE_GROUP, GS, R, blocks, RBLOCK, smem);
    return true;
}

inline bool plan_fast(long long B, int m_max, int d, const ReduceEnv& env, ReduceLaunch& L, bool& complete) {
    complete = false;
    if (m_max < 1 || m_max > 64 || d < 1 || d > 16) return false;
    if (d <= 4 && m_max <= 32) {
        const long long minb = d == 4 ? (m_max >= 14 ? PLP_REDUCE_LANE4_MINB_ROWS14 : PLP_REDUCE_LANE4_MINB) : PLP_REDUCE_LANE_MINB;
        const bool other = env.split || env.half;
        if (is(env.lane, '1') || (!is(env.lane, '0') && !other && B > minb)) {
            complete = true;
            return plan_lane(B, m_max, d, env, L);
        }
    }
    if (d > 8) {
        if (is(env.r2, '0')) return false;
        if (is(env.r1, '1') && m_max > 32) return plan_group(B, d, 64, 1, env, L);
        const bool small_batch = !env.lazy && B <= PLP_REDUCE_WG_MAXB && !(env.r1 && env.r1[0]);
        if (is(env.lazy, '1') || (m_max > 32 && !is(env.lazy, '0')) || small_batch) return plan_lazy(B, d, env, L, complete);
        return plan_group(B, d, m_max <= 32 ? 16 : 32, 2, env, L);
    }
    const int gs = group_size_r(m_max);
    if (d >= 5) {
        const bool small_batch = !env.lazy && B <= PLP_REDUCE_WG_MAXB && !env.split && !env.half;
        if (is(env.lazy, '1') || (m_max > 32 && !is(env.lazy, '0')) || small_batch) return plan_lazy(B, d, env, L, complete);
        const bool latency_form = is(env.split, '1') || (!is(env.split, '0') && B <= PLP_REDUCE_SPLIT_MAXB(d, gs));
        if (!latency_form) return plan_group(B, d, m_max <= 16 ? 8 : (m_max <= 32 ? 16 : 32), 2, env, L);
    }
    return plan_group(B, d, gs, 4, env, L);
}

}

inline ReducePlan plan_reduce(long long B, int m_max, int d, const ReduceEnv& env) {
    using namespace plan_detail;
    ReducePlan p;
    if (m_max < 0 || m_max > 64 || d < 1 || d > 16) return p;
    p.force_retry = is(env.retry_all, '1') ? 1 : 0;
    const int gs = reduce_general_gs(m_max);
    long long blocks = cdiv(B, REDUCE_GENERAL_BLOCK / gs);
    if (blocks > (1ll << 20)) blocks = 1ll << 20;
    blocks = at_least1(blocks);
    p.retry = launch(RE_GENERAL, gs, 1, blocks > 256 * 8 ? 256 * 8 : blocks, REDUCE_GENERAL_BLOCK, reduce_smem_bytes(gs, d));
    p.first = p.retry;
    p.first.grid = blocks;
    bool complete = false;
    ReduceLaunch fast;
    if (is(env.one_row, '1') || !plan_fast(B, m_max, d, env, fast, complete)) return p;
    p.first = fast;
    p.second = !complete;
    return p;
}

}
```

Before: 13.41 billion.

## Repack surviving lane LPs into multi-lane groups mid-solve in reduce lane engine

Splits the lane simplex walks into begin/pass steps. Between passes, the wave ballots which LPs are still unsolved, and when few remain it compacts them into pairs or quads of lanes so each LP's row scan is split across more lanes. Finished results are parked and shuffled back to their original lanes at the end. The aim is to cut the long tail where a handful of slow LPs keep the whole wave busy with mostly idle lanes. In exchange it adds shuffle and state-migration overhead plus extra register pressure, and it is enabled by default with an env switch to turn it off.

```diff
diff --git a/polytope_amd/csrc/plp_bbox_lane.hip b/polytope_amd/csrc/plp_bbox_lane.hip
--- a/polytope_amd/csrc/plp_bbox_lane.hip
+++ b/polytope_amd/csrc/plp_bbox_lane.hip
@@ -1,4 +1,5 @@
 #include "plp_reduce_lane.hpp"
+#include "plp_reduce_plan.hpp"
 
 namespace plp {
 
@@ -7,6 +8,7 @@
                               int* status, hipStream_t st, double* xfin) {
     if (B > 2147483647ll) return 1;
     const int force = 0;
+    const int repack = reduce_lane_repack(reduce_env());
     const bool wide = m_max > LN_ROWS;
     int gs = wide ? (B <= PLP_REDUCE_LANE32_GS16_MAXB ? 16 : 8) : (B <= PLP_REDUCE_LANE_GS16_MAXB ? 16 : (B <= PLP_REDUCE_LANE_GS8_MAXB ? 8 : 4));
     const long long ng = 64 / gs;
@@ -14,7 +16,7 @@
     if (blocks < 1) blocks = 1;
 #define PLP_BBL(GSV, RV)                                                                                                     \
     hipLaunchKernelGGL((bbox_lane_kernel<D, GSV, RV>), dim3((unsigned)blocks), dim3(RBLOCK), reduce_lane_smem_bytes(D, GSV, RV), st, B, \
-                       m_max, A, b, mrows, force, lb, ub, status, xfin)
+                       m_max, A, b, mrows, force, repack, lb, ub, status, xfin)
     if (wide) { if (gs == 16) PLP_BBL(16, 32); else PLP_BBL(8, 32); }
     else if (gs == 16) PLP_BBL(16, 16);
     else if (gs == 8) PLP_BBL(8, 16);
diff --git a/polytope_amd/csrc/plp_kernels.hpp b/polytope_amd/csrc/plp_kernels.hpp
--- a/polytope_amd/csrc/plp_kernels.hpp
+++ b/polytope_amd/csrc/plp_kernels.hpp
@@ -95,6 +95,7 @@
     unsigned long long* ctr;
     unsigned long long* retry_word;
     unsigned long long epoch;
+    int repack = 1;
 };
 int launch_reduce(int d, const ReduceArgs& a, int phase, hipStream_t st);
 
diff --git a/polytope_amd/csrc/plp_lane_lp.hpp b/polytope_amd/csrc/plp_lane_lp.hpp
--- a/polytope_amd/csrc/plp_lane_lp.hpp
+++ b/polytope_amd/csrc/plp_lane_lp.hpp
@@ -63,9 +63,9 @@
 
 constexpr double LANE_PAIR_SIN2 = 1e-10;
 
-template <class RowF, class RatioF, class Ratio0F, class AnyF>
-PLP_LANE_FN void walk3(Lp3& S, const double c0, const double c1, const double c2, const bool go, RowF ROWS, RatioF RATIO,
-                       Ratio0F RATIO0, AnyF ANY, const bool warm = false) {
+template <class Ratio0F, class AnyF>
+PLP_LANE_FN void walk3_begin(Lp3& S, const double c0, const double c1, const double c2, const bool go, Ratio0F RATIO0, AnyF ANY,
+                             const bool warm = false) {
     if (!warm) {
         S.x0 = S.x1 = S.x2 = 0.0;
         S.w0 = S.w1 = S.w2 = -1;
@@ -98,7 +98,12 @@
             }
         }
     }
-    while (ANY(S.status < 0)) {
+}
+
+template <class RowF, class RatioF, class AnyF>
+PLP_LANE_FN void walk3_pass(Lp3& S, const double c0, const double c1, const double c2, RowF ROWS, RatioF RATIO, AnyF ANY) {
+    const double cn1 = fabs(c0) + fabs(c1) + fabs(c2);
+    {
         const bool run = S.status < 0;
         double d0 = -c0, d1 = -c1, d2 = -c2;
         double n00 = 0, n01 = 0, n02 = 0, n10 = 0, n11 = 0, n12 = 0, n20 = 0, n21 = 0, n22 = 0;
@@ -214,6 +219,13 @@
     }
 }
 
+template <class RowF, class RatioF, class Ratio0F, class AnyF>
+PLP_LANE_FN void walk3(Lp3& S, const double c0, const double c1, const double c2, const bool go, RowF ROWS, RatioF RATIO,
+                       Ratio0F RATIO0, AnyF ANY, const bool warm = false) {
+    walk3_begin(S, c0, c1, c2, go, RATIO0, ANY, warm);
+    while (ANY(S.status < 0)) walk3_pass(S, c0, c1, c2, ROWS, RATIO, ANY);
+}
+
 template <class RowF, class RatioF, class AnyF>
 PLP_LANE_FN void walk3(Lp3& S, const double c0, const double c1, const double c2, const bool go, RowF ROWS, RatioF RATIO,
                        AnyF ANY, const bool warm = false) {
@@ -244,9 +256,7 @@
     e3 = -fma(p0, m12, fma(-p1, m02, p2 * m01));
 }
 
-template <class RowF, class RatioF, class AnyF>
-PLP_LANE_FN void walk4(Lp4& S, const double c0, const double c1, const double c2, const double c3, const bool go, RowF ROWS,
-                       RatioF RATIO, AnyF ANY) {
+PLP_LANE_FN void walk4_begin(Lp4& S, const double c0, const double c1, const double c2, const double c3, const bool go) {
     S.x0 = S.x1 = S.x2 = S.x3 = 0.0;
     S.w0 = S.w1 = S.w2 = S.w3 = -1;
     S.nact = 0;
@@ -255,7 +265,13 @@
     S.status = go ? -1 : ST_OPT;
     const double cn1 = fabs(c0) + fabs(c1) + fabs(c2) + fabs(c3);
     if (go && !(cn1 > 0.0)) S.status = ST_OPT;
-    while (ANY(S.status < 0)) {
+}
+
+template <class RowF, class RatioF, class AnyF>
+PLP_LANE_FN void walk4_pass(Lp4& S, const double c0, const double c1, const double c2, const double c3, RowF ROWS, RatioF RATIO,
+                            AnyF ANY) {
+    const double cn1 = fabs(c0) + fabs(c1) + fabs(c2) + fabs(c3);
+    {
         const bool run = S.status < 0;
         bool dropped = false;
         double d0 = -c0, d1 = -c1, d2 = -c2, d3 = -c3;
@@ -436,6 +452,13 @@
     }
 }
 
+template <class RowF, class RatioF, class AnyF>
+PLP_LANE_FN void walk4(Lp4& S, const double c0, const double c1, const double c2, const double c3, const bool go, RowF ROWS,
+                       RatioF RATIO, AnyF ANY) {
+    walk4_begin(S, c0, c1, c2, c3, go);
+    while (ANY(S.status < 0)) walk4_pass(S, c0, c1, c2, c3, ROWS, RATIO, ANY);
+}
+
 PLP_LANE_FN void ratio_row4(const double a0, const double a1, const double a2, const double a3, const double beta, const int i,
                             const double d0, const double d1, const double d2, const double d3, const double x0,
                             const double x1, const double x2, const double x3, const double tolp, double& bs, double& bd,
diff --git a/polytope_amd/csrc/plp_reduce.hip b/polytope_amd/csrc/plp_reduce.hip
--- a/polytope_amd/csrc/plp_reduce.hip
+++ b/polytope_amd/csrc/plp_reduce.hip
@@ -17,9 +17,11 @@
     }
 }
 
-int launch_reduce(int d, const ReduceArgs& a, int phase, hipStream_t st) {
-    const ReducePlan p = plan_reduce(a.B, a.m_max, d, reduce_env());
+int launch_reduce(int d, const ReduceArgs& args, int phase, hipStream_t st) {
+    const ReducePlan p = plan_reduce(args.B, args.m_max, d, reduce_env());
     if (p.first.engine == RE_NONE) return 2;
+    ReduceArgs a = args;
+    a.repack = p.lane_repack;
     if (phase != 2) {
         const int rc = launch_plan(d, p.first, a, p.force_retry, 0, st);
         if (rc || !p.second || phase == 1) return rc;
diff --git a/polytope_amd/csrc/plp_reduce_d1_4.hip b/polytope_amd/csrc/plp_reduce_d1_4.hip
--- a/polytope_amd/csrc/plp_reduce_d1_4.hip
+++ b/polytope_amd/csrc/plp_reduce_d1_4.hip
@@ -20,3 +20,15 @@
     return 0;
 }
 #endif
+
+#ifdef PLP_LANE_DBG_HIST
+extern "C" __attribute__((visibility("default"))) int plp_debug_lane_hist(unsigned long long* out, int reset) {
+    (void)hipDeviceSynchronize();
+    if (out && hipMemcpyFromSymbol(out, HIP_SYMBOL(plp::plp_lane_hist), sizeof(plp::plp_lane_hist)) != hipSuccess) return 1;
+    if (reset) {
+        static const unsigned long long z[9 * 16 * 4] = {0};
+        if (hipMemcpyToSymbol(HIP_SYMBOL(plp::plp_lane_hist), z, sizeof(z)) != hipSuccess) return 1;
+    }
+    return 0;
+}
+#endif
diff --git a/polytope_amd/csrc/plp_reduce_lane.hpp b/polytope_amd/csrc/plp_reduce_lane.hpp
--- a/polytope_amd/csrc/plp_reduce_lane.hpp
+++ b/polytope_amd/csrc/plp_reduce_lane.hpp
@@ -9,6 +9,17 @@
 
 #ifndef PLP_LANE_CH
 #define PLP_LANE_CH 4
+#endif
+
+#ifndef PLP_LANE_REPACK_PAIR
+#define PLP_LANE_REPACK_PAIR 32
+#endif
+#ifndef PLP_LANE_REPACK_QUAD
+#define PLP_LANE_REPACK_QUAD 16
+#endif
+
+#ifdef PLP_LANE_DBG_HIST
+static __device__ unsigned long long plp_lane_hist[9][16][4];
 #endif
 
 constexpr int LN_ROWS = 16;
@@ -37,7 +48,7 @@
 template <int D, int GS, int ROWS = LN_ROWS, bool BBOX = false>
 __device__ __forceinline__ void reduce_lane_tile(
     const long long tile, long long B, int m_max, const double* __restrict__ Ag, const double* __restrict__ bg,
-    const int* __restrict__ mrows, double abs_tol, int force_retry, unsigned long long* __restrict__ keep_out,
+    const int* __restrict__ mrows, double abs_tol, int force_retry, int repack, unsigned long long* __restrict__ keep_out,
     int* __restrict__ flags_out, double* __restrict__ r_out, double* __restrict__ xc_out, int* __restrict__ nlp_out,
     unsigned long long* __restrict__ ctr) {
     static_assert(D >= 1 && D <= 4, "the lane engine walks in R^3 (lower dimensions are embedded) or R^4");
@@ -273,6 +284,7 @@
     int nlp = 1;
     uint64_t keep = 0ull;
     int stage = 0;
+    int ncert = 0;
     if (fulldim) {
         const int neq = __popcll(live);
         if (neq <= D + 1) { flags = RF_EARLY; keep = live; }
@@ -282,11 +294,16 @@
     __syncthreads();
     auto any_lane = [](bool p) { return __any(p) != 0; };
     using LpState = std::conditional_t<D == 4, lane::Lp4, lane::Lp3>;
-    auto lane_solve = [&](LpState& S, const double (&cv)[4], const bool go_, const double* pA, const double* pbeta, auto relax_tag,
-                          int krv, const int nparts, const int part) {
+    auto lane_solve = [&](const double (&cv0)[4], const bool go_, const int tp0, auto relax_tag, const int krv0, const int nparts0,
+                          auto nq_tag, auto FIN, const int kind, int& st, double (&q)[decltype(nq_tag)::value]) {
         constexpr bool RELAX = decltype(relax_tag)::value;
-        const int cnt = rows / nparts;
-        const int i0 = part * cnt;
+        constexpr int NQ = decltype(nq_tag)::value;
+        LpState S;
+        double cv[4] = {cv0[0], cv0[1], cv0[2], cv0[3]};
+        int krv = krv0, nparts = nparts0;
+        int cnt = rows / nparts;
+        int i0 = (lane & (nparts - 1)) * cnt;
+        const double* pA = sA + tp0;
         auto row_of = [&](const double* base, double& a0, double& a1, double& a2, double& a3) {
             a0 = base[0];
             a1 = D > 1 ? base[(D > 1 ? 1 : 0) * LS] : 0.0;
@@ -297,7 +314,7 @@
             constexpr bool X0 = decltype(x0_tag)::value;
             if constexpr (RELAX) asm volatile("" : "+v"(krv));
             const double* ra = pA + i0 * D * LS;
-            const double* rb_ = pbeta + i0 * LS;
+            const double* rb_ = pA + OFF_N + i0 * LS;
             int ic = i0;
             for (int ch = 0; ch < cnt; ch += PLP_LANE_CH) {
 #pragma unroll
@@ -331,32 +348,132 @@
             if (nparts > 1) meet(std::integral_constant<int, PLP_DPP_XOR1>{});
             if (nparts > 2) meet(std::integral_constant<int, PLP_DPP_XOR2>{});
         };
+        auto one_pass = [&]() {
+            if constexpr (D == 4) {
+                lane::walk4_pass(
+                    S, cv[0], cv[1], cv[2], cv[3],
+                    [&](int i, double& a0, double& a1, double& a2, double& a3) { row_of(pA + (i * D) * LS, a0, a1, a2, a3); },
+                    [&](double d0, double d1, double d2, double d3, double x0, double x1, double x2, double x3, double tolp, double& bs,
+                        double& bd, int& bi) {
+                        const double dv[4] = {d0, d1, d2, d3}, xv[4] = {x0, x1, x2, x3};
+                        ratio(std::false_type{}, dv, xv, tolp, bs, bd, bi);
+                    },
+                    any_lane);
+            } else {
+                lane::walk3_pass(
+                    S, cv[0], cv[1], cv[2],
+                    [&](int i, double& a0, double& a1, double& a2) {
+                        double a3;
+                        row_of(pA + (i * D) * LS, a0, a1, a2, a3);
+                    },
+                    [&](double d0, double d1, double d2, double x0, double x1, double x2, double tolp, double& bs, double& bd, int& bi) {
+                        const double dv[4] = {d0, d1, d2, 0.0}, xv[4] = {x0, x1, x2, 0.0};
+                        ratio(std::false_type{}, dv, xv, tolp, bs, bd, bi);
+                    },
+                    any_lane);
+            }
+        };
+#ifdef PLP_LANE_DBG_HIST
+        int npass = 0;
+        auto hist = [&](int n) {
+            if (lane == 0) {
+                unsigned long long* h = plp_lane_hist[(GS == 4 ? 0 : (GS == 8 ? 3 : 6)) + kind][npass < 15 ? npass : 15];
+                atomicAdd(h, 1ull);
+                atomicAdd(h + 1, (unsigned long long)n);
+                atomicAdd(h + 2, n <= 32 ? 1ull : 0ull);
+                atomicAdd(h + 3, n <= 16 ? 1ull : 0ull);
+            }
+            ++npass;
+        };
+        hist(__popcll(__ballot(go_)) / nparts);
+#else
+        (void)kind;
+#endif
         if constexpr (D == 4) {
-            lane::walk4(
-                S, cv[0], cv[1], cv[2], cv[3], go_,
-                [&](int i, double& a0, double& a1, double& a2, double& a3) { row_of(pA + (i * D) * LS, a0, a1, a2, a3); },
-                [&](double d0, double d1, double d2, double d3, double x0, double x1, double x2, double x3, double tolp, double& bs,
-                    double& bd, int& bi) {
-                    const double dv[4] = {d0, d1, d2, d3}, xv[4] = {x0, x1, x2, x3};
-                    ratio(std::false_type{}, dv, xv, tolp, bs, bd, bi);
-                },
-                any_lane);
+            lane::walk4_begin(S, cv[0], cv[1], cv[2], cv[3], go_);
         } else {
-            lane::walk3(
+            lane::walk3_begin(
                 S, cv[0], cv[1], cv[2], go_,
-                [&](int i, double& a0, double& a1, double& a2) {
-                    double a3;
-                    row_of(pA + (i * D) * LS, a0, a1, a2, a3);
-                },
-                [&](double d0, double d1, double d2, double x0, double x1, double x2, double tolp, double& bs, double& bd, int& bi) {
-                    const double dv[4] = {d0, d1, d2, 0.0}, xv[4] = {x0, x1, x2, 0.0};
-                    ratio(std::false_type{}, dv, xv, tolp, bs, bd, bi);
-                },
                 [&](double d0, double d1, double d2, double tolp, double& bs, double& bd, int& bi) {
                     const double dv[4] = {d0, d1, d2, 0.0}, xv[4] = {0.0, 0.0, 0.0, 0.0};
                     ratio(std::true_type{}, dv, xv, tolp, bs, bd, bi);
                 },
                 any_lane);
+        }
+        int where = lane & ~(nparts - 1);
+        bool moved = false;
+        int hst = 0;
+        double hq[NQ];
+#pragma unroll
+        for (int k = 0; k < NQ; ++k) hq[k] = 0.0;
+        int tp = tp0;
+        for (;;) {
+            const uint64_t un = __ballot(S.status < 0);
+            if (un == 0ull) break;
+#ifdef PLP_LANE_DBG_HIST
+            hist(__popcll(un) / nparts);
+#endif
+            if (repack && nparts < 4) {
+                const uint64_t low = nparts == 1 ? un : (un & 0x5555555555555555ull);
+                const int n = __popcll(low);
+                const int np_new = n <= PLP_LANE_REPACK_QUAD ? 4 : ((nparts == 1 && n <= PLP_LANE_REPACK_PAIR) ? 2 : nparts);
+                if (np_new != nparts) {
+                    const int sh = np_new == 4 ? 2 : 1;
+                    double fq[NQ];
+                    FIN(S, cv, krv, fq);
+                    {
+                        const int from = where < 0 ? lane : where;
+                        const int fs = __shfl(S.status, from, 64);
+                        const bool park = (where >= 0) & (fs >= 0);
+                        hst = park ? fs : hst;
+#pragma unroll
+                        for (int k = 0; k < NQ; ++k) {
+                            const double t = __shfl(fq[k], from, 64);
+                            hq[k] = park ? t : hq[k];
+                        }
+                        const int rank = __popcll(low & ((1ull << (from & 63)) - 1ull));
+                        where = ((where < 0) | park) ? -1 : (rank << sh);
+                    }
+                    const bool src = ((low >> lane) & 1ull) != 0ull;
+                    const int rank_s = __popcll(low & ((1ull << lane) - 1ull));
+                    int from = __builtin_amdgcn_ds_permute((src ? (rank_s << sh) : 1) << 2, lane);
+                    from = __shfl(from, lane & ~(np_new - 1), 64);
+                    const bool holds = (lane >> sh) < n;
+                    from = holds ? from : lane;
+                    auto mv_i = [&](int& v) { v = __shfl(v, from, 64); };
+                    auto mv_d = [&](double& v) { v = __shfl(v, from, 64); };
+                    mv_d(S.x0); mv_d(S.x1); mv_d(S.x2);
+                    mv_i(S.w0); mv_i(S.w1); mv_i(S.w2);
+                    if constexpr (D == 4) { mv_d(S.x3); mv_i(S.w3); }
+                    mv_i(S.nact); mv_i(S.status); mv_i(S.iters); mv_i(S.ndeg);
+#pragma unroll
+                    for (int k = 0; k < (D == 4 ? 4 : 3); ++k) mv_d(cv[k]);
+                    mv_i(tp);
+                    mv_i(krv);
+                    S.status = holds ? S.status : (int)ST_OPT;
+                    pA = sA + tp;
+                    nparts = np_new;
+                    cnt = rows / nparts;
+                    i0 = (lane & (nparts - 1)) * cnt;
+                    moved = true;
+                }
+            }
+            one_pass();
+        }
+        double fq[NQ];
+        FIN(S, cv, krv, fq);
+        st = S.status;
+#pragma unroll
+        for (int k = 0; k < NQ; ++k) q[k] = fq[k];
+        if (moved) {
+            const int from = where < 0 ? lane : where;
+            const int fs = __shfl(S.status, from, 64);
+            st = where < 0 ? hst : fs;
+#pragma unroll
+            for (int k = 0; k < NQ; ++k) {
+                const double t = __shfl(fq[k], from, 64);
+                q[k] = where < 0 ? hq[k] : t;
+            }
         }
     };
     auto x_of_lp = [](const LpState& S, int k) {
@@ -390,23 +507,38 @@
             const int kx = it >> 1;
             const bool up = it & 1;
             const double cs = up ? -1.0 : 1.0;
-            LpState S;
             const double cv[4] = {kx == 0 ? cs : 0.0, kx == 1 ? cs : 0.0, kx == 2 ? cs : 0.0, kx == 3 ? cs : 0.0};
-            lane_solve(S, cv, mine, myA, myan, std::false_type{}, -1, nparts, part);
+            constexpr int NQ3 = BBOX ? D : 1;
+            int status;
+            double xq[NQ3];
+            lane_solve(cv, mine, gib, std::false_type{}, kx, nparts, std::integral_constant<int, NQ3>{},
+                       [&](const LpState& S_, const double (&)[4], const int k_, double (&o)[NQ3]) {
+                           if constexpr (BBOX) {
+#pragma unroll
+                               for (int kk = 0; kk < D; ++kk) o[kk] = x_of_lp(S_, kk);
+                           } else {
+                               o[0] = x_of_lp(S_, k_);
+                           }
+                       },
+                       rd, status, xq);
             double xck = 0.0;
 #pragma unroll
             for (int kk = 0; kk < D; ++kk) xck = (kk == kx) ? xc[kk] : xck;
-            const double xk = x_of_lp(S, kx);
+            double xk = xq[0];
+            if constexpr (BBOX) {
+#pragma unroll
+                for (int kk = 1; kk < D; ++kk) xk = (kk == (kx < D ? kx : D - 1)) ? xq[kk] : xk;
+            }
             double v;
-            if (S.status == ST_OPT) v = xck + xk;
-            else if (S.status == ST_UNBND) v = up ? pinf : -pinf;
-            else { v = qnan; lpfail = lpfail | (mine & (S.status != ST_RETRY)); }
-            retry = retry | (mine & (S.status == ST_RETRY));
+            if (status == ST_OPT) v = xck + xk;
+            else if (status == ST_UNBND) v = up ? pinf : -pinf;
+            else { v = qnan; lpfail = lpfail | (mine & (status != ST_RETRY)); }
+            retry = retry | (mine & (status == ST_RETRY));
             if constexpr (BBOX) {
                 double* xfin = reinterpret_cast<double*>(keep_out);
                 if (xfin && (valid & mine & (part == 0))) {
 #pragma unroll
-                    for (int kk = 0; kk < D; ++kk) xfin[((size_t)(tile + gib) * 2 * D + it) * D + kk] = xc[kk] + x_of_lp(S, kk);
+                    for (int kk = 0; kk < D; ++kk) xfin[((size_t)(tile + gib) * 2 * D + it) * D + kk] = xc[kk] + xq[kk < NQ3 ? kk : 0];
                 }
             }
 #pragma unroll
@@ -480,7 +612,7 @@
             for (int k = 0; k < R; ++k) cert |= spread_rows<R, GS>(grp_ballot(((okb >> k) & 1u) != 0u, g)) << k;
             keep |= cert;
             todo &= ~cert;
-            ctr_add(ctr, -__popcll(cert), g.gl == 0);
+            ncert = __popcll(cert);
         }
 #endif
         __syncthreads();
@@ -505,7 +637,6 @@
             const int sh = nparts == 4 ? 2 : (nparts == 2 ? 1 : 0);
             const int per = 64 >> sh;
             const int t = rb + (lane >> sh);
-            const int part = lane & (nparts - 1);
             int tp = 0, toff = 0, run = 0;
             unsigned ttd = 0u;
             for (int p = 0; p < NG; ++p) {
@@ -528,17 +659,21 @@
             double c[4] = {0.0, 0.0, 0.0, 0.0};
 #pragma unroll
             for (int kk = 0; kk < D; ++kk) c[kk] = -pA[(kr * D + kk) * LS];
-            LpState S;
-            lane_solve(S, c, mine, pA, pan, std::true_type{}, kr, nparts, part);
-            double akx = -lane::dot3(c[0], c[1], c[2], S.x0, S.x1, S.x2);
-            if constexpr (D == 4) akx = -lane::dot4(c[0], c[1], c[2], c[3], S.x0, S.x1, S.x2, S.x3);
-            const double obj = akx - pan[kr * LS];
-            const bool keepk = mine & (((S.status == ST_OPT) & (obj > abs_tol)) | (S.status == ST_UNBND));
+            int status;
+            double akxq[1];
+            lane_solve(c, mine, tp, std::true_type{}, kr, nparts, std::integral_constant<int, 1>{},
+                       [&](const LpState& S_, const double (&c_)[4], const int, double (&o)[1]) {
+                           if constexpr (D == 4) o[0] = -lane::dot4(c_[0], c_[1], c_[2], c_[3], S_.x0, S_.x1, S_.x2, S_.x3);
+                           else o[0] = -lane::dot3(c_[0], c_[1], c_[2], S_.x0, S_.x1, S_.x2);
+                       },
+                       2, status, akxq);
+            const double obj = akxq[0] - pan[kr * LS];
+            const bool keepk = mine & (((status == ST_OPT) & (obj > abs_tol)) | (status == ST_UNBND));
             const uint64_t all = __ballot(keepk);
-            const uint64_t rt = __ballot(mine & (S.status == ST_RETRY));
+            const uint64_t rt = __ballot(mine & (status == ST_RETRY));
             if (rt != 0ull) {
                 for (int p = 0; p < NG; ++p)
-                    if (__any(mine & (S.status == ST_RETRY) & (tp == p))) retry_polys |= 1u << p;
+                    if (__any(mine & (status == ST_RETRY) & (tp == p))) retry_polys |= 1u << p;
             }
 #pragma unroll
             for (int k = 0; k < R; ++k) {
@@ -558,7 +693,7 @@
         (flags_out + tile)[gib] = flags;
         (nlp_out + tile)[gib] = nlp;
     }
-    ctr_add(ctr, nlp, valid & (g.gl == 0));
+    ctr_add(ctr, (valid ? nlp : 0) - ncert, g.gl == 0);
     const uint64_t rb64 = __ballot(retry & valid & (g.gl == 0));
     if (rb64 != 0ull) {
         __threadfence_block();
@@ -581,32 +716,33 @@
 template <int D, int GS, int ROWS = LN_ROWS>
 __global__ __launch_bounds__(RBLOCK, PLP_REDUCE_LANE_WAVES(D)) void reduce_lane_kernel(
     long long B, int m_max, const double* __restrict__ Ag, const double* __restrict__ bg, const int* __restrict__ mrows,
-    double abs_tol, int force_retry, unsigned long long* __restrict__ keep_out, int* __restrict__ flags_out,
+    double abs_tol, int force_retry, int repack, unsigned long long* __restrict__ keep_out, int* __restrict__ flags_out,
     double* __restrict__ r_out, double* __restrict__ xc_out, int* __restrict__ nlp_out, unsigned long long* __restrict__ ctr) {
-    reduce_lane_tile<D, GS, ROWS>((long long)blockIdx.x * (64 / GS), B, m_max, Ag, bg, mrows, abs_tol, force_retry, keep_out,
+    reduce_lane_tile<D, GS, ROWS>((long long)blockIdx.x * (64 / GS), B, m_max, Ag, bg, mrows, abs_tol, force_retry, repack, keep_out,
                                   flags_out, r_out, xc_out, nlp_out, ctr);
 }
 
 template <int D, int ROWS, int GSA, int GSB>
 __global__ __launch_bounds__(RBLOCK, PLP_REDUCE_LANE_WAVES(D)) void reduce_lane_mix_kernel(
     int nbig, long long B, int m_max, const double* __restrict__ Ag, const double* __restrict__ bg,
-    const int* __restrict__ mrows, double abs_tol, int force_retry, unsigned long long* __restrict__ keep_out,
+    const int* __restrict__ mrows, double abs_tol, int force_retry, int repack, unsigned long long* __restrict__ keep_out,
     int* __restrict__ flags_out, double* __restrict__ r_out, double* __restrict__ xc_out, int* __restrict__ nlp_out,
     unsigned long long* __restrict__ ctr) {
     constexpr int NA = 64 / GSA, NB_ = 64 / GSB;
     if ((int)blockIdx.x < nbig)
-        reduce_lane_tile<D, GSA, ROWS>((long long)blockIdx.x * NA, B, m_max, Ag, bg, mrows, abs_tol, force_retry, keep_out,
+        reduce_lane_tile<D, GSA, ROWS>((long long)blockIdx.x * NA, B, m_max, Ag, bg, mrows, abs_tol, force_retry, repack, keep_out,
                                        flags_out, r_out, xc_out, nlp_out, ctr);
     else
         reduce_lane_tile<D, GSB, ROWS>((long long)nbig * NA + (long long)((int)blockIdx.x - nbig) * NB_, B, m_max, Ag, bg, mrows,
-                                       abs_tol, force_retry, keep_out, flags_out, r_out, xc_out, nlp_out, ctr);
+                                       abs_tol, force_retry, repack, keep_out, flags_out, r_out, xc_out, nlp_out, ctr);
 }
 
 template <int D, int GS, int ROWS>
 __global__ __launch_bounds__(RBLOCK, PLP_REDUCE_LANE_WAVES(D)) void bbox_lane_kernel(
     long long B, int m_max, const double* __restrict__ Ag, const double* __restrict__ bg, const int* __restrict__ mrows,
-    int force_retry, double* __restrict__ lb, double* __restrict__ ub, int* __restrict__ status, double* __restrict__ xfin) {
-    reduce_lane_tile<D, GS, ROWS, true>((long long)blockIdx.x * (64 / GS), B, m_max, Ag, bg, mrows, 0.0, force_retry,
+    int force_retry, int repack, double* __restrict__ lb, double* __restrict__ ub, int* __restrict__ status,
+    double* __restrict__ xfin) {
+    reduce_lane_tile<D, GS, ROWS, true>((long long)blockIdx.x * (64 / GS), B, m_max, Ag, bg, mrows, 0.0, force_retry, repack,
                                         reinterpret_cast<unsigned long long*>(xfin), status, lb, ub, nullptr, nullptr);
 }
 
diff --git a/polytope_amd/csrc/plp_reduce_launch.hpp b/polytope_amd/csrc/plp_reduce_launch.hpp
--- a/polytope_amd/csrc/plp_reduce_launch.hpp
+++ b/polytope_amd/csrc/plp_reduce_launch.hpp
@@ -22,7 +22,7 @@
 
 #define PLP_REDUCE_GO_LANE(KERNEL)                                                                                              \
     hipLaunchKernelGGL(KERNEL, dim3((unsigned)L.grid), dim3(L.block), L.lds, st, a.B, a.m_max, a.A, a.b, a.mrows, a.abs_tol, \
-                       force, a.keep, a.flags, a.r, a.xc, a.nlp, a.ctr)
+                       force, a.repack, a.keep, a.flags, a.r, a.xc, a.nlp, a.ctr)
 
 template <int D>
 int launch_reduce_d(const ReduceLaunch& L, const ReduceArgs& a, int force, int retry_only, hipStream_t st) {
@@ -49,11 +49,11 @@
             if constexpr (D <= 4) {
                 if (L.rows == 32)
                     hipLaunchKernelGGL((reduce_lane_mix_kernel<D, 32, 8, 16>), dim3((unsigned)L.grid), dim3(L.block), L.lds, st,
-                                       (int)L.nbig, a.B, a.m_max, a.A, a.b, a.mrows, a.abs_tol, force, a.keep, a.flags, a.r, a.xc,
+                                       (int)L.nbig, a.B, a.m_max, a.A, a.b, a.mrows, a.abs_tol, force, a.repack, a.keep, a.flags, a.r, a.xc,
                                        a.nlp, a.ctr);
                 else
                     hipLaunchKernelGGL((reduce_lane_mix_kernel<D, 16, 4, 8>), dim3((unsigned)L.grid), dim3(L.block), L.lds, st,
-                                       (int)L.nbig, a.B, a.m_max, a.A, a.b, a.mrows, a.abs_tol, force, a.keep, a.flags, a.r, a.xc,
+                                       (int)L.nbig, a.B, a.m_max, a.A, a.b, a.mrows, a.abs_tol, force, a.repack, a.keep, a.flags, a.r, a.xc,
                                        a.nlp, a.ctr);
                 return 0;
             }
diff --git a/polytope_amd/csrc/plp_reduce_plan.hpp b/polytope_amd/csrc/plp_reduce_plan.hpp
--- a/polytope_amd/csrc/plp_reduce_plan.hpp
+++ b/polytope_amd/csrc/plp_reduce_plan.hpp
@@ -108,6 +108,7 @@
     bool second = false;
     ReduceLaunch retry;
     int force_retry = 0;
+    int lane_repack = 1;
 };
 
 struct ReduceEnv {
@@ -123,6 +124,7 @@
     const char* half = nullptr;
     const char* wsplit = nullptr;
     const char* wdense = nullptr;
+    const char* lane_repack = nullptr;
 };
 
 inline ReduceEnv reduce_env() {
@@ -139,8 +141,11 @@
     e.half = getenv("PLP_REDUCE_HALF");
     e.wsplit = getenv("PLP_REDUCE_WSPLIT");
     e.wdense = getenv("PLP_REDUCE_WDENSE");
+    e.lane_repack = getenv("PLP_REDUCE_LANE_REPACK");
     return e;
 }
+
+inline int reduce_lane_repack(const ReduceEnv& e) { return (e.lane_repack && e.lane_repack[0] == '0') ? 0 : 1; }
 
 namespace plan_detail {
 
@@ -274,6 +279,7 @@
     ReducePlan p;
     if (m_max < 0 || m_max > 64 || d < 1 || d > 16) return p;
     p.force_retry = is(env.retry_all, '1') ? 1 : 0;
+    p.lane_repack = reduce_lane_repack(env);
     const int gs = reduce_general_gs(m_max);
     long long blocks = cdiv(B, REDUCE_GENERAL_BLOCK / gs);
     if (blocks > (1ll << 20)) blocks = 1ll << 20;
```

Result: no change. 13.39 billion (-0.1%).
